# joaotavora/raytracing-one-weekend

Hardware: AMD Instinct MI355X
Metric: Msamples/sec (W×H×spp) on cover scene; achieved HBM GB/s vs peak (higher is better)
Workload: dtype f64

## Files before the change

### include/rtow.h

```cpp
#ifndef RTOW_H
#define RTOW_H

#include <stdint.h>

#ifdef __cplusplus
extern "C" {
#endif

#define RTOW_ABI_VERSION 9

#define RTOW_OK 0
#define RTOW_EINVAL (-1)
#define RTOW_ENODEV (-2)
#define RTOW_EHIP (-3)
#define RTOW_ENOSCENE (-4)
#define RTOW_EEMPTY (-5)
#define RTOW_ENOMEM (-6)

#define RTOW_MAT_LAMBERTIAN 0
#define RTOW_MAT_METAL 1
#define RTOW_MAT_DIELECTRIC 2

#define RTOW_PRIM_SPHERE 0
#define RTOW_PRIM_MOVING_SPHERE 1
// ... 51 lines not shown
  const int32_t *prim_index;
} rtow_scene_t;

typedef struct rtow_config_t {
  int32_t image_width;
  int32_t image_height;
  int32_t samples_per_pixel;
  int32_t nstreams;
  int32_t max_child_rays;
  int32_t precision;
  int32_t kernel;
  int32_t rank;
  int32_t nranks;
  int32_t tile_rows;
  uint64_t seed;
  int32_t stream_first;
  int32_t stream_count;
  int32_t accumulate;
  int32_t pad_;
} rtow_config_t;

typedef struct rtow_stats_t {
  uint64_t samples;
  uint64_t segments;
  uint64_t prim_tests;
  uint64_t node_tests;
  double kernel_ms;
  double total_ms;
  int32_t local_rows;
  int32_t kernel_used;
} rtow_stats_t;

typedef struct rtow_ctx rtow_ctx;

int rtow_abi_version(void);
const char *rtow_last_error(void);

int rtow_ctx_create(int device_id, rtow_ctx **out);
void rtow_ctx_destroy(rtow_ctx *ctx);

int rtow_scene_upload(rtow_ctx *ctx, const rtow_scene_t *scene);

#define RTOW_BUILDER_HOST_SAH 0
#define RTOW_BUILDER_DEVICE_LBVH 1
#define RTOW_BUILDER_AUTO 2
int rtow_ctx_set_builder(rtow_ctx *ctx, int32_t builder);

typedef struct rtow_build_info_t {
  int32_t builder;
  int32_t bvh_nodes;
  int32_t bvh_image_bytes;
  int32_t grid_image_bytes;
  double bvh_build_ms;
  double grid_build_ms;
  double upload_ms;
  int32_t bvh4_nodes;
  int32_t bvh4_image_bytes;
  int32_t ref_tree_nodes;
  int32_t bvh4_node_bytes;
  double ref_tree_stupid_volume;
  double ref_tree_build_ms;
} rtow_build_info_t;
int rtow_build_info(rtow_ctx *ctx, rtow_build_info_t *out);

int rtow_local_rows(const rtow_config_t *cfg);
int rtow_local_row_list(const rtow_config_t *cfg, int32_t *rows_out, int32_t capacity);

int rtow_render_device(rtow_ctx *ctx, const rtow_config_t *cfg, void *d_rgb_sums,
                       void *hip_stream, rtow_stats_t *stats);

int rtow_render_device_rgb8(rtow_ctx *ctx, const rtow_config_t *cfg, void *d_rgb8, void *hip_stream,
                            rtow_stats_t *stats);

int rtow_tonemap_device(rtow_ctx *ctx, const void *d_rgb_sums, int64_t n_values, int32_t spp_effective,
                        void *d_rgb8, void *hip_stream);

int rtow_profile_collect(rtow_ctx *ctx, double *kernel_ms_sum, int32_t *launches);

int rtow_debug_counters(rtow_ctx *ctx, unsigned long long *out48);

int rtow_debug_schedule(rtow_ctx *ctx, const rtow_config_t *cfg, uint32_t *out_pairs, int32_t capacity_pairs);

int rtow_debug_last_spec(rtow_ctx *ctx, uint32_t *out_spec);

int rtow_debug_tile_order(const rtow_scene_t *scene, const rtow_config_t *cfg, uint32_t *table_out, unsigned char *empty_out,
                          int32_t capacity, int32_t *n_empty, int32_t *tile_w_log2, int32_t *tile_h_log2);

int rtow_debug_image(rtow_ctx *ctx, int32_t which, void *out, int64_t capacity, int64_t *size_out);

typedef struct rtow_ray_t {
  double origin[3];
  double time;
  double direction[3];
  double tmax;
} rtow_ray_t;

typedef struct rtow_hit_t {
  double t;
  double point[3];
  double normal[3];
  int32_t prim;
  int32_t kind;
  int32_t material;
  int32_t front_face;
} rtow_hit_t;

int rtow_intersect_device(rtow_ctx *ctx, int32_t precision, int32_t kernel, const void *d_rays, int64_t n_rays,
                          void *d_hits, void *hip_stream, rtow_stats_t *stats);
int rtow_intersect(rtow_ctx *ctx, int32_t precision, int32_t kernel, const rtow_ray_t *rays, int64_t n_rays,
                   rtow_hit_t *hits, rtow_stats_t *stats);

int rtow_occluded_device(rtow_ctx *ctx, int32_t precision, int32_t kernel, const void *d_rays, int64_t n_rays,
                         void *d_occluded , void *hip_stream, rtow_stats_t *stats);
int rtow_occluded(rtow_ctx *ctx, int32_t precision, int32_t kernel, const rtow_ray_t *rays, int64_t n_rays,
                  uint8_t *occluded, rtow_stats_t *stats);

#define RTOW_MAX_HITS 8
int rtow_first_hits_device(rtow_ctx *ctx, int32_t precision, int32_t kernel, const void *d_rays, int64_t n_rays,
                           int32_t max_hits, void *d_hits ,
                           void *d_counts , void *hip_stream, rtow_stats_t *stats);
int rtow_first_hits(rtow_ctx *ctx, int32_t precision, int32_t kernel, const rtow_ray_t *rays, int64_t n_rays,
                    int32_t max_hits, rtow_hit_t *hits, int32_t *counts , rtow_stats_t *stats);

typedef struct rtow_point_query_t {
  double point[3];
  double time;
  double max_dist;
  double pad_;
} rtow_point_query_t;

typedef struct rtow_point_hit_t {
  double dist;
  double point[3];
  int32_t prim;
  int32_t kind;
  int32_t material;
  int32_t pad_;
} rtow_point_hit_t;

int rtow_closest_point_device(rtow_ctx *ctx, int32_t precision, int32_t kernel, const void *d_queries, int64_t n,
                              void *d_hits, void *hip_stream, rtow_stats_t *stats);
int rtow_closest_point(rtow_ctx *ctx, int32_t precision, int32_t kernel, const rtow_point_query_t *queries, int64_t n,
                       rtow_point_hit_t *hits, rtow_stats_t *stats);

#define RTOW_MAX_NEAREST 8
int rtow_nearest_device(rtow_ctx *ctx, int32_t precision, int32_t kernel, const void *d_queries, int64_t n,
                        int32_t k, void *d_hits , void *d_counts ,
                        void *hip_stream, rtow_stats_t *stats);
int rtow_nearest(rtow_ctx *ctx, int32_t precision, int32_t kernel, const rtow_point_query_t *queries, int64_t n,
                 int32_t k, rtow_point_hit_t *hits, int32_t *counts , rtow_stats_t *stats);

typedef struct rtow_radiance_params_t {
  uint64_t seed;
  int32_t samples_per_ray;
  int32_t max_child_rays;
  uint32_t sample_first;
  int32_t pad_;
} rtow_radiance_params_t;

int rtow_radiance_device(rtow_ctx *ctx, int32_t precision, int32_t kernel, const rtow_radiance_params_t *params,
                         const void *d_rays, int64_t n_rays, const void *d_ids ,
                         void *d_rgb_sums , void *hip_stream, rtow_stats_t *stats);
int rtow_radiance(rtow_ctx *ctx, int32_t precision, int32_t kernel, const rtow_radiance_params_t *params,
                  const rtow_ray_t *rays, int64_t n_rays, const uint32_t *ids, double *rgb_sums, rtow_stats_t *stats);

typedef struct rtow_guide_t {
// ... 83 lines not shown
```

### raytracing-one-weekend_amd/csrc/rtow_capi.cpp

```cpp

#include "rtow_ctx.h"

namespace {

thread_local std::string g_err;

template <class F>
int guarded(const char *what, F &&f) noexcept {
  try {
    return f();
  } catch (const std::bad_alloc &) {
    return fail(RTOW_ENOMEM, "%s: out of host memory", what);
  } catch (const std::exception &e) {
    return fail(RTOW_EINVAL, "%s: %s", what, e.what());
  } catch (...) {
    return fail(RTOW_EINVAL, "%s: unknown C++ exception", what);
  }
}

}
namespace rtow {
int set_last_error(int code, const char *fmt, ...) {
  char buf[512];
  va_list ap;
// ... 703 lines not shown
  P.local_rows = rows;
  P.seed_lo = (uint32_t)cfg->seed;
  P.seed_hi = (uint32_t)(cfg->seed >> 32);
  P.n_items = (uint32_t)n_items;
  P.n_lanes = (uint32_t)n_lanes;
  P.npix_local = (uint32_t)npix;
  P.div_npix = make_fastdiv((uint32_t)npix);
  P.div_w = make_fastdiv((uint32_t)cfg->image_width);
  P.div_tile = make_fastdiv((uint32_t)cfg->tile_rows);
  P.div_ns = make_fastdiv((uint32_t)streams_now);
  uint32_t th = 0, tw = 0;
  if (!c->knobs.no_tiles) tile_shape(cfg, rows, th, tw);
  P.tile_h_log2 = th;
  P.tile_w_log2 = tw;
  P.div_tpr_n = th ? (uint32_t)cfg->image_width >> tw : 1u;
  P.div_tpr = make_fastdiv(P.div_tpr_n);
  P.n_tile_rows = th ? (uint32_t)rows >> th : 1u;
  P.tile_table = nullptr;
  P.n_items_first = P.n_items;
  P.empty_batch = 64u;
  if (th) {
    const uint32_t sky_rows = P.n_tile_rows * (uint32_t)c->knobs.sky_eighths / 8u;
    const long long key[10] = {1, c->scene_gen, cfg->image_width, cfg->image_height, cfg->rank, cfg->nranks, cfg->tile_rows,
                               (long long)th, (long long)sky_rows, c->knobs.tile_order ? 1 : 0};
    if (std::memcmp(key, c->tile_key, sizeof key) != 0) {
      std::vector<unsigned char> empty;
      std::vector<uint32_t> table;
      if (c->knobs.tile_order) tile_classify(c->host_scene, cfg, th, tw, rows, empty);
      c->tile_empty = tile_queue_table(empty, c->knobs.tile_order, P.div_tpr_n, P.n_tile_rows, sky_rows, table);
      if ((rc = c->tile_table.ensure(table.size() * sizeof(uint32_t)))) return rc;
      c->tile_key[0] = -1;
      HIPCHK(hipStreamSynchronize(st));
      HIPCHK(hipMemcpy(c->tile_table.p, table.data(), table.size() * sizeof(uint32_t), hipMemcpyHostToDevice));
      std::memcpy(c->tile_key, key, sizeof key);
    }
    P.tile_table = (const uint32_t *)c->tile_table.p;
    P.n_items_first = P.n_items - c->tile_empty * 64u * (uint32_t)streams_now;
    P.empty_batch = 64u * (uint32_t)c->knobs.empty_levels;
  }
  P.partials = (double *)c->partials.p;
  P.stack = (uint32_t *)c->stack.p;
  P.spill = (uint32_t *)c->spill.p;
  P.spec = rtow::kSpecGeneric;
  if (kernel == RTOW_KERNEL_GRID && lds_bytes > 0 && !f32 && !c->knobs.no_spec && scene.n_tri == 0) {
    if (scene.n_mov == 0 && c->grid_fat_stride == 48u) P.spec = rtow::kSpecStaticSpheres;
    if (scene.n_mov > 0 && c->grid_fat_stride == 80u) P.spec = rtow::kSpecMovingSpheres;
    if (P.spec != rtow::kSpecGeneric && c->grid_ny == 1 && !c->knobs.no_flat) P.spec |= rtow::kSpecFlatY;
  }
  P.walk = c->grid_walk;
  P.b4_trips = c->knobs.bvh4_sm ? 0u : 1u;
  {
    const bool b4 = kernel == RTOW_KERNEL_BVH4;
    const bool b4_nodes_resident = b4 && scene.b4_lds_limit >= scene.b4_off_tri;
    int cap = c->knobs.walk_cap, open = c->knobs.walk_max_open;
    if (cap < 0) {
      cap = b4 ? 4 : 3;
      open = b4 ? (b4_nodes_resident ? 24 : 32) : 16;
    }
    if (cap > 0 && !b4) cap = std::max(cap, 3);
    P.walk_cap = cap > 0 ? (uint32_t)cap : 0xffffffffu;
    P.walk_max_open = (uint32_t)open;
    P.leaf_votes = (uint32_t)(c->knobs.leaf_votes > 0 ? c->knobs.leaf_votes : (b4 ? 28 : 16));
  }
  P.fetch_votes = (uint32_t)(c->knobs.fetch_votes > 0 ? c->knobs.fetch_votes : (kernel == RTOW_KERNEL_BVH4 ? 2 : 4));
  P.sm4_restart = (uint32_t)c->knobs.sm4_votes[0];
  P.sm4_scatter = (uint32_t)c->knobs.sm4_votes[1];
  P.sm4_leaf = (uint32_t)c->knobs.sm4_votes[2];
  P.counters = (unsigned long long *)c->counters.p;
  P.t_origin = P.counters + 16;

  if (st != nullptr) HIPCHK(hipStreamWaitEvent(st, c->upload_ev, 0));
  if (stats) HIPCHK(hipEventRecord(c->call_ev[0], st));
  if (!c->counters_init.p) {
    std::vector<unsigned long long> init(48, 0ull);
    init[5] = init[16] = ~0ull;
    if ((rc = c->counters_init.ensure(48 * sizeof(unsigned long long)))) return rc;
    HIPCHK(hipMemcpy(c->counters_init.p, init.data(), 48 * sizeof(unsigned long long), hipMemcpyHostToDevice));
  }
  HIPCHK(hipMemcpyAsync(c->counters.p, c->counters_init.p, 48 * sizeof(unsigned long long), hipMemcpyDeviceToDevice, st));
  const int slot = c->ev_count < kEventRing ? c->ev_count : -1;
  if (slot >= 0) HIPCHK(hipEventRecord(c->ev[slot][0], st));
  int launch_kernel = kernel;
  if (image_kernel && lds_bytes > 0 && c->knobs.stamps) launch_kernel = kernel + 16;
  int lrc = strict ? rtow::launch_trace_strict(P, launch_kernel, (int)grid, block, lds_bytes, st)
            : f32  ? rtow::launch_trace_f32(P, launch_kernel, (int)grid, block, lds_bytes, st)
                   : rtow::launch_trace_fast(P, launch_kernel, (int)grid, block, lds_bytes, st);
#ifdef RTOW_TAILSTAT
  if (const char *path = std::getenv("RTOW_TAILSTAT_OUT")) {
    HIPCHK(hipStreamSynchronize(st));
    std::vector<unsigned long long> ts((size_t)n_lanes / 64 * 8);
    HIPCHK(hipMemcpy(ts.data(), c->spill.p, ts.size() * 8, hipMemcpyDeviceToHost));
    if (FILE *f = std::fopen(path, "wb")) {
      std::fwrite(ts.data(), 8, ts.size(), f);
      std::fclose(f);
    }
  }
#endif
  if (lrc != 0) return fail(RTOW_EHIP, "trace kernel launch failed: %s", hipGetErrorString((hipError_t)lrc));
  c->last_spec = (int64_t)P.spec;
  if (slot >= 0) {
    HIPCHK(hipEventRecord(c->ev[slot][1], st));
    c->ev_count++;
  }
  rtow::ReduceParams R;
  R.partials = P.partials;
  R.out = (double *)d_rgb_sums;
  R.npix3 = (uint32_t)(npix * 3);
  R.nstreams = streams_now;
  R.accumulate = accumulate;
  R.W = (uint32_t)cfg->image_width;
  R.tile_w_log2 = tw;
  R.tile_h_log2 = th;
  R.tiles_per_row = P.div_tpr_n;
  R.rgb8 = nullptr;
  R.spp = 0.0;
  if (c->fuse_rgb8 && lvl_first == 0 && lvl_count == plan.count && !accumulate) {
    R.rgb8 = c->fuse_rgb8;
    R.spp = c->fuse_spp;
    c->fuse_used = true;
  }
  lrc = rtow::launch_reduce(R, st);
  if (lrc != 0) return fail(RTOW_EHIP, "reduce kernel launch failed: %s", hipGetErrorString((hipError_t)lrc));

  if (stats) {
    HIPCHK(hipEventRecord(c->call_ev[1], st));
    HIPCHK(hipMemcpyAsync(c->h_counters, c->counters.p, 48 * sizeof(unsigned long long),
                          hipMemcpyDeviceToHost, st));
    HIPCHK(hipStreamSynchronize(st));
    if (c->h_counters[47] != 0ull) {
      (void)check_dropped(c, false);
      return fail(RTOW_EHIP, "trace kernel: end-of-launch bound reached, %llu lanes gave up their samples",
                  c->h_counters[47]);
    }
    float ms = 0.f;
    HIPCHK(hipEventElapsedTime(&ms, c->call_ev[0], c->call_ev[1]));
    stats->total_ms = ms;
    if (slot >= 0) {
      HIPCHK(hipEventElapsedTime(&ms, c->ev[slot][0], c->ev[slot][1]));
      stats->kernel_ms = ms;
    }
    stats->samples = npix * ((unsigned long long)spt * (unsigned long long)(streams_now - 1) + (unsigned long long)spt_last);
    stats->segments = c->h_counters[1];
    if (kernel == RTOW_KERNEL_BRUTE) {
      stats->prim_tests = stats->segments * (unsigned long long)c->n_prims;
      stats->node_tests = 0;
    } else {
      stats->prim_tests = c->h_counters[2];
      stats->node_tests = c->h_counters[3];
    }
  }
  return RTOW_OK;
}

constexpr int64_t kMaxQueryRays = (1ll << 31) - 64;

static int query_map(rtow_ctx *c, int which, const int32_t **out) {
  if (c->q_map_ok[which]) {
    *out = (const int32_t *)c->q_map[which].p;
    return RTOW_OK;
  }
  const int ns = c->ds.n_sph, nm = c->ds.n_mov, nt = c->ds.n_tri, np = c->n_prims;
  const rtow_ctx::HostSceneCopy &h = c->host_scene;
  std::vector<int32_t> cls2ins((size_t)np);
  for (int i = 0; i < np; ++i) cls2ins[i] = i;
  if (h.have_order)
    for (int i = 0; i < np; ++i) {
      const int k = h.pk[i];
      const int base = k == RTOW_PRIM_SPHERE ? 0 : (k == RTOW_PRIM_MOVING_SPHERE ? ns : ns + nm);
      cls2ins[(size_t)base + h.pi[i]] = i;
    }
  std::vector<int32_t> table;
  if (which == 0) {
    table.swap(cls2ins);
  } else {
    std::vector<int32_t> matched;
    if (!c->rf.ready)
      if (int rc = match_slots(c, which, matched)) return rc;
    const std::vector<int32_t> &slot2tri = c->rf.ready ? c->rf.slot2tri[which - 1] : matched;
    table.assign((size_t)nt, -1);
    for (int k = 0; k < nt; ++k) table[(size_t)k] = cls2ins[(size_t)ns + nm + slot2tri[(size_t)k]];
  }
  DevBuf &b = c->q_map[which];
// ... 422 lines not shown
  HIPCHK(hipSetDevice(c->device));
  if ((rc = c->q_rays.ensure((size_t)n * sizeof(rtow_ray_t))) || (ids && (rc = c->q_ids.ensure((size_t)n * 8)))) return rc;
  if ((rc = camera_rays_device(c, cfg, c->q_rays.p, ids ? c->q_ids.p : nullptr, nullptr))) return rc;
  HIPCHK(hipMemcpy(rays, c->q_rays.p, (size_t)n * sizeof(rtow_ray_t), hipMemcpyDeviceToHost));
  if (ids) HIPCHK(hipMemcpy(ids, c->q_ids.p, (size_t)n * 8, hipMemcpyDeviceToHost));
  return RTOW_OK;
}

static int guides_device(rtow_ctx *c, const rtow_config_t *cfg, void *d_guides, void *hip_stream, rtow_stats_t *stats) {
  if (!c) return fail(RTOW_EINVAL, "ctx is NULL");
  CameraCall k;
  int rc;
  if ((rc = camera_call(cfg, k))) return rc;
  const long long tiles = (((long long)cfg->image_width + 7) / 8) * (((long long)k.rows + 7) / 8);
  if (tiles * 64 > 0xfffffff0LL) return fail(RTOW_EINVAL, "too many pixels (%lld)", k.npix);
  if (k.npix > 0 && !d_guides) return fail(RTOW_EINVAL, "NULL guide buffer");
  if (((uintptr_t)d_guides & 15u) != 0u) return fail(RTOW_EINVAL, "guide buffer must be 16-byte aligned");
  QueryRun q;
  if ((rc = query_begin(c, cfg->precision, cfg->kernel, stats, q))) return rc;
  if (stats) stats->local_rows = k.rows;
  if (k.npix == 0) return RTOW_OK;
  if (k.samples == 0) {
    HIPCHK(hipMemsetAsync(d_guides, 0, (size_t)k.npix * sizeof(rtow_guide_t), (hipStream_t)hip_stream));
    if (stats) HIPCHK(hipStreamSynchronize((hipStream_t)hip_stream));
    return RTOW_OK;
  }
  q.block_cap = c->knobs.guides_blocks;

  const int kernel = q.kernel;
  const int block = q.shape.block;
  const unsigned lds = q.shape.lds_bytes;
  const int build = q.strict ? 0 : 1;
  rtow::GuidesLaunchFn *const launch[2] = {rtow::launch_guides_strict, rtow::launch_guides_fast};
  rtow::QueryOccupancyFn *const occupancy[2] = {rtow::guides_occupancy_strict, rtow::guides_occupancy_fast};
  const int occ = occupancy[build](kernel, block, lds, nullptr);
  rc = query_launch(c, q, tiles * 64, occ, hip_stream, stats, [&](const rtow::TraceParams &P0, unsigned long long *counters, int grid) {
    rtow::TraceParams P = P0;
    camera_params(c, cfg, k, P);
    return launch[build](P, d_guides, (uint32_t)(tiles * 64), k.sample_first, (int32_t)k.samples, counters, kernel, grid, block,
                         lds, hip_stream);
  });
  if (rc == RTOW_OK && stats) {
    stats->samples = stats->segments = (uint64_t)k.npix * (uint64_t)k.samples;
    if (kernel == RTOW_KERNEL_BRUTE) stats->prim_tests = stats->segments * (uint64_t)c->n_prims;
  }
  return rc;
}

static int guides_host(rtow_ctx *c, const rtow_config_t *cfg, rtow_guide_t *guides, rtow_stats_t *stats) {
  if (!c) return fail(RTOW_EINVAL, "ctx is NULL");
  CameraCall k;
  int rc;
  if ((rc = camera_call(cfg, k))) return rc;
  if (k.npix > 0 && !guides) return fail(RTOW_EINVAL, "NULL guide array");
  if (k.npix == 0) return guides_device(c, cfg, nullptr, nullptr, stats);
  if (!c->have_scene) return fail(RTOW_ENOSCENE, "no scene uploaded");
  HIPCHK(hipSetDevice(c->device));
  if ((rc = c->q_guides.ensure((size_t)k.npix * sizeof(rtow_guide_t)))) return rc;
  if ((rc = guides_device(c, cfg, c->q_guides.p, nullptr, stats))) return rc;
  HIPCHK(hipMemcpy(guides, c->q_guides.p, (size_t)k.npix * sizeof(rtow_guide_t), hipMemcpyDeviceToHost));
  return RTOW_OK;
}
static_assert(sizeof(rtow_guide_t) == 64, "rtow_guide_t is four 16-byte stores");

int64_t rtow_camera_ray_count(const rtow_config_t *cfg) {
  CameraCall k;
  if (int rc = camera_call(cfg, k)) return rc;
  return (int64_t)(k.npix * k.samples);
}

int rtow_debug_counters(rtow_ctx *c, unsigned long long *out48) {
  if (!c || !out48) return fail(RTOW_EINVAL, "NULL argument");
  if (!c->counters.p) return fail(RTOW_ENOSCENE, "no launch yet");
  HIPCHK(hipSetDevice(c->device));
  HIPCHK(hipDeviceSynchronize());
  HIPCHK(hipMemcpy(out48, c->counters.p, 48 * sizeof(unsigned long long), hipMemcpyDeviceToHost));
  return RTOW_OK;
}

int rtow_debug_last_spec(rtow_ctx *c, uint32_t *out_spec) {
  if (!c || !out_spec) return fail(RTOW_EINVAL, "NULL argument");
  if (c->last_spec < 0) return fail(RTOW_ENOSCENE, "no launch yet");
  *out_spec = (uint32_t)c->last_spec;
  return RTOW_OK;
}

int rtow_tonemap_device(rtow_ctx *c, const void *d_rgb_sums, int64_t n_values, int32_t spp_effective,
                        void *d_rgb8, void *hip_stream) {
  if (!c) return fail(RTOW_EINVAL, "ctx is NULL");
  if (!d_rgb_sums || !d_rgb8) return fail(RTOW_EINVAL, "NULL device pointer");
  if (n_values < 0 || n_values > 0xffffffffLL) return fail(RTOW_EINVAL, "n_values out of range");
  if (spp_effective <= 0) return fail(RTOW_EINVAL, "spp_effective must be positive");
  HIPCHK(hipSetDevice(c->device));
  int lrc = rtow::launch_tonemap((const double *)d_rgb_sums, (unsigned char *)d_rgb8, (uint32_t)n_values,
                                 (double)spp_effective, hip_stream);
  if (lrc != 0) return fail(RTOW_EHIP, "tonemap launch failed: %s", hipGetErrorString((hipError_t)lrc));
  return RTOW_OK;
}

int rtow_profile_collect(rtow_ctx *c, double *kernel_ms_sum, int32_t *launches) {
  if (!c) return fail(RTOW_EINVAL, "ctx is NULL");
  HIPCHK(hipSetDevice(c->device));
  double sum = 0.0;
  for (int i = 0; i < c->ev_count; ++i) {
    HIPCHK(hipEventSynchronize(c->ev[i][1]));
    float ms = 0.f;
    HIPCHK(hipEventElapsedTime(&ms, c->ev[i][0], c->ev[i][1]));
    sum += ms;
  }
  if (kernel_ms_sum) *kernel_ms_sum = sum;
  if (launches) *launches = c->ev_count;
  const bool waited = c->ev_count > 0;
  c->ev_count = 0;
  return waited ? check_dropped(c, false) : RTOW_OK;
}

static int impl_render(rtow_ctx *c, const rtow_scene_t *scene, const rtow_config_t *cfg, double *rgb_sums_host,
                rtow_stats_t *stats) {
  if (!c) return fail(RTOW_EINVAL, "ctx is NULL");
  if (!rgb_sums_host) return fail(RTOW_EINVAL, "rgb_sums_host is NULL");
  int rc = validate_cfg(cfg);
  if (rc) return rc;
  if ((rc = upload_for(c, scene, cfg))) return rc;
  const int rows = rtow_local_rows(cfg);
  const size_t bytes = (size_t)rows * cfg->image_width * 3 * sizeof(double);
  if (bytes == 0) {
    if (stats) {
      std::memset(stats, 0, sizeof *stats);
    }
    return RTOW_OK;
  }
  if ((rc = c->out.ensure(bytes))) return rc;
  void *d_out = c->out.p;
  if (cfg->accumulate)
    HIPCHK(hipMemcpy(d_out, rgb_sums_host, bytes, hipMemcpyHostToDevice));
  rc = rtow_render_device(c, cfg, d_out, nullptr, stats);
  if (rc != RTOW_OK) return rc;
  if ((rc = mirror_dropped(c, nullptr))) return rc;
  HIPCHK(hipMemcpy(rgb_sums_host, d_out, bytes, hipMemcpyDeviceToHost));
  return check_dropped(c, true);
}

static int impl_render_device_rgb8(rtow_ctx *c, const rtow_config_t *cfg, void *d_rgb8, void *hip_stream,
                                   rtow_stats_t *stats) {
  if (!c) return fail(RTOW_EINVAL, "ctx is NULL");
  if (!d_rgb8) return fail(RTOW_EINVAL, "d_rgb8 is NULL");
  int rc = validate_cfg(cfg);
  if (rc) return rc;
  const int spp_eff = cfg->samples_per_pixel / cfg->nstreams * cfg->nstreams;
  if (spp_eff <= 0) return fail(RTOW_EINVAL, "no effective samples (samples_per_pixel < nstreams)");
  if (cfg->accumulate) return fail(RTOW_EINVAL, "the rgb8 entry points own their sums: accumulate must be 0");
  const int rows = rtow_local_rows(cfg);
  const size_t n = (size_t)rows * cfg->image_width * 3;
  if (n == 0) {
    if (stats) std::memset(stats, 0, sizeof *stats);
    return RTOW_OK;
  }
  HIPCHK(hipSetDevice(c->device));
  if ((rc = c->out.ensure(n * sizeof(double)))) return rc;
  c->fuse_rgb8 = (unsigned char *)d_rgb8;
  c->fuse_spp = (double)spp_eff;
  c->fuse_used = false;
  rc = impl_render_device(c, cfg, c->out.p, hip_stream, stats);
  c->fuse_rgb8 = nullptr;
  if (rc == RTOW_OK && !c->fuse_used) rc = rtow_tonemap_device(c, c->out.p, (int64_t)n, spp_eff, d_rgb8, hip_stream);
  return rc;
// ... 168 lines not shown
```

### raytracing-one-weekend_amd/csrc/rtow_ctx.h

```cpp
#pragma once
#include <hip/hip_runtime.h>

#include <cmath>
#include <cstdarg>
#include <cstdio>
#include <cstdlib>
#include <algorithm>
#include <chrono>
#include <cstring>
#include <string>
#include <vector>

#include "../../include/rtow.h"
#include "rtow_bvh.h"
#include "rtow_bvh4.h"
#include "rtow_device.h"
#include "rtow_grid.h"
#include "rtow_reftree.h"

namespace rtow {
int set_last_error(int code, const char *fmt, ...);
template <class... A>
inline int fail(int code, const char *fmt, A... a) {
  return set_last_error(code, fmt, a...);
// ... 8 lines not shown
      return fail(RTOW_EHIP, "%s: %s (%s:%d)", #expr, hipGetErrorString(e_), __FILE__, __LINE__); \
  } while (0)

constexpr unsigned kLdsLimit = 160u * 1024u;
constexpr int kEventRing = 256;

namespace rtow {

struct DevBuf {
  void *p = nullptr;
  size_t bytes = 0;
  int ensure(size_t need) {
    if (need <= bytes) return RTOW_OK;
    if (p) {
      HIPCHK(hipFree(p));
      p = nullptr;
      bytes = 0;
    }
    size_t want = need + need / 8 + 256;
    HIPCHK(hipMalloc(&p, want));
    bytes = want;
    return RTOW_OK;
  }
  void release() {
    if (p) (void)hipFree(p);
    p = nullptr;
    bytes = 0;
  }
};

struct PinnedArena {
  unsigned char *p = nullptr;
  size_t cap = 0, used = 0;
};
int h2d_block(void *dst, const void *src, size_t n);

template <class T>
int upload(DevBuf &b, const std::vector<T> &v) {
  const size_t n = v.size() * sizeof(T);
  if (int rc = b.ensure(n ? n : sizeof(T))) return rc;
  return n ? h2d_block(b.p, v.data(), n) : RTOW_OK;
}

inline double now_ms() {
  using namespace std::chrono;
  return duration<double, std::milli>(steady_clock::now().time_since_epoch()).count();
}

}
using rtow::DevBuf;
using rtow::PinnedArena;
using rtow::h2d_block;
using rtow::now_ms;
using rtow::upload;

struct Knobs {
  int bvh_leaf = 0;
  double bvh_ct = -1.0;
  bool no_leaf_order = false;
  double grid_cpp = 1.0;
  double grid_large = 4.0;
  int grid_max_tris = 8192;
  unsigned long long partials_cap = 8ull << 30;
  int bvh_block = 0;
  int blocks_per_cu = 0;
  bool no_tiles = false;
  int sky_eighths = 1;
  bool stamps = false;
  bool bvh4_no_aux = false;
  bool no_bvh4 = false;
  int fetch_votes = 0;
  int leaf_votes = 0;
  int walk_cap = -1, walk_max_open = 0;
  bool bvh4_sm = false;
  int sm4_votes[3] = {8, 16, 16};
  int bvh4_stack_k = 0;
  int sched_chunk = 10;
  int sched_chunk_mesh = 16;
  int ploc_radius = -1;
  int device_tree = 2;
  bool stream_scalar = false;
  bool no_spec = false;
  bool no_flat = false;
  bool tile_order = true;
  int empty_levels = 3;
  int tail_bound = 0;
  int radiance_blocks = 0;
  int guides_blocks = 0;
  void read() {
    auto geti = [](const char *n, int d) { const char *e = std::getenv(n); return e ? std::atoi(e) : d; };
    auto getd = [](const char *n, double d) { const char *e = std::getenv(n); return e ? std::atof(e) : d; };
    bvh_leaf = geti("RTOW_BVH_LEAF", 0);
    bvh_ct = getd("RTOW_BVH_CT", -1.0);
    no_leaf_order = std::getenv("RTOW_NO_LEAF_ORDER") != nullptr;
    grid_cpp = getd("RTOW_GRID_CPP", 1.0);
    grid_large = getd("RTOW_GRID_LARGE", 4.0);
    grid_max_tris = geti("RTOW_GRID_MAX_TRIS", 8192);
    if (const char *e = std::getenv("RTOW_PARTIALS_MAX_MB")) partials_cap = (unsigned long long)std::atoll(e) << 20;
    bvh_block = geti("RTOW_BVH_BLOCK", 0);
    if (bvh_block != 256 && bvh_block != 512 && bvh_block != 1024) bvh_block = 0;
    blocks_per_cu = geti("RTOW_BLOCKS_PER_CU", 0);
    if (blocks_per_cu < 1 || blocks_per_cu > 16) blocks_per_cu = 0;
    no_tiles = std::getenv("RTOW_NO_TILES") != nullptr;
    sky_eighths = std::min(std::max(geti("RTOW_SKY_EIGHTHS", 1), 0), 8);
    stamps = std::getenv("RTOW_STAMPS") != nullptr;
    no_bvh4 = std::getenv("RTOW_NO_BVH4") != nullptr;
    bvh4_no_aux = std::getenv("RTOW_BVH4_NO_AUX") != nullptr;
    fetch_votes = std::min(std::max(geti("RTOW_FETCH_VOTES", 0), 0), 64);
    leaf_votes = std::min(std::max(geti("RTOW_LEAF_VOTES", 0), 0), 64);
    bvh4_sm = std::getenv("RTOW_BVH4_SM") != nullptr;
    if (const char *e = std::getenv("RTOW_WALK_CAP")) {
      int a = 0, b = 0;
      if (std::sscanf(e, "%d,%d", &a, &b) == 2 && a > 0 && b > 0) {
        walk_cap = a;
        walk_max_open = std::min(b, 64);
      } else {
        walk_cap = 0;
      }
    }
    if (const char *e = std::getenv("RTOW_SM4_VOTES")) {
      int a = 0, b = 0, d = 0;
      if (std::sscanf(e, "%d,%d,%d", &a, &b, &d) == 3) {
        sm4_votes[0] = std::min(std::max(a, 1), 64);
        sm4_votes[1] = std::min(std::max(b, 1), 64);
        sm4_votes[2] = std::min(std::max(d, 1), 64);
      }
    }
    bvh4_stack_k = std::min(std::max(geti("RTOW_BVH4_STACK_K", 0), 0), 64);
    sched_chunk = std::min(std::max(geti("RTOW_SCHED_CHUNK", 10), 0), 4096);
    sched_chunk_mesh = std::min(std::max(geti("RTOW_SCHED_CHUNK_MESH", 16), 0), 4096);
    tail_bound = std::max(geti("RTOW_TAIL_BOUND", 0), 0);
    radiance_blocks = std::max(geti("RTOW_RADIANCE_BLOCKS", 0), 0);
    guides_blocks = std::max(geti("RTOW_GUIDES_BLOCKS", 0), 0);
    tile_order = geti("RTOW_TILE_ORDER", 1) != 0;
    empty_levels = std::min(std::max(geti("RTOW_EMPTY_LEVELS", 3), 1), 16);
    no_spec = std::getenv("RTOW_NO_SPEC") != nullptr;
    no_flat = std::getenv("RTOW_NO_FLAT") != nullptr;
    stream_scalar = std::getenv("RTOW_STREAM_SCALAR") != nullptr;
    if (const char *e = std::getenv("RTOW_PLOC_RADIUS")) ploc_radius = std::min(std::max(std::atoi(e), 0), 64);
    if (const char *e = std::getenv("RTOW_DEVICE_TREE"))
      device_tree = std::strcmp(e, "radix") == 0 ? 0 : (std::strcmp(e, "ploc") == 0 ? 1 : 2);
    if (ploc_radius >= 0 && !std::getenv("RTOW_DEVICE_TREE")) device_tree = ploc_radius == 0 ? 0 : 1;
  }
};

constexpr unsigned kNeedBvh = 1u, kNeedGrid = 2u, kNeedF32 = 4u, kNeedBvh4 = 8u, kNeedAll = 15u;

struct rtow_ctx {
  int device = 0;
  Knobs knobs;
  int num_cus = 0;
  bool have_scene = false;
  rtow::DevScene ds{};
  rtow::DevCamera cam{};
  int n_prims = 0;
  DevBuf sph, sph_r, mov, tri, tri16, prim_mat, mats, blob, cam_dev, gblob;
  DevBuf blob4;
  bool have_bvh4 = false;
  bool have_tri16 = false;
  int bvh4_depth = 0;
  DevBuf blob32, gblob32, cam32_dev;
  rtow::DevScene ds32{};
  uint32_t gblob_bytes = 0;
  uint32_t grid_fat_stride = 0;
  int32_t grid_ny = 0;
  GridWalkConsts grid_walk{};
  int64_t last_spec = -1;
  bool have_grid = false;
  uint32_t blob_bytes = 0;
  long long bvh_nodes = 0;
  int builder = RTOW_BUILDER_HOST_SAH;
  int builder_req = RTOW_BUILDER_AUTO;
  void *lbvh_scratch = nullptr;
  void *grid_scratch = nullptr;
  rtow_build_info_t build_info{};
  struct HostSceneCopy {
    std::vector<double> sg, mg, tg;
    std::vector<int32_t> pk, pi;
    bool have_order = false;
    rtow_camera_t cam{};
  } host_scene;
  DevBuf tile_table;
  long long tile_key[10] = {-1, 0, 0, 0, 0, 0, 0, 0, 0, 0};
  uint32_t tile_empty = 0;
  long long scene_gen = 0;
  DevBuf rtree;
  bool have_rtree = false;
  PinnedArena arena;
  unsigned built = 0;
  DevBuf partials, stack, counters, spill;
  DevBuf out, out8;
  unsigned char *fuse_rgb8 = nullptr;
  double fuse_spp = 0.0;
  bool fuse_used = false;
  DevBuf counters_init;
  DevBuf dropped;
  unsigned long long *h_dropped = nullptr;
  hipEvent_t upload_ev = nullptr;
  int occ[3][5] = {{0, 0, 0, 0, 0}, {0, 0, 0, 0, 0}, {0, 0, 0, 0, 0}};
  hipEvent_t ev[kEventRing][2] = {};
  int ev_count = 0;
  hipEvent_t call_ev[2] = {};
  unsigned long long *h_counters = nullptr;
  DevBuf q_counters, q_spill, q_rays, q_hits, q_occ, q_map[3];
  DevBuf q_stack, q_ids, q_rgb;
  DevBuf q_guides;
  DevBuf q_khits, q_kcounts;
  bool q_map_ok[3] = {false, false, false};
  hipEvent_t q_ev[4] = {};
  unsigned long long *h_qcounters = nullptr;
  struct Refit {
    bool ready = false;
    std::vector<int32_t> slot2tri[2];
    DevBuf map2, map4, par2, par4, need4, flags, nbox2, nbox4, sbox4, pbox, partials;
    DevBuf area;
    DevBuf g_sph, g_mov, g_tri;
    int refits = 0;
    double refit_ms = 0.0;
    hipEvent_t ev[2] = {};
  } rf;
};

static uint32_t bvh4_min_stack(const rtow_ctx *c) { return c->knobs.bvh4_stack_k > 0 ? (uint32_t)c->knobs.bvh4_stack_k : 6u; }

namespace rtow {
void lbvh_release(void *handle);
void grid_build_release(void *handle);
int validate_scene(const rtow_scene_t *s);
int impl_scene_upload(rtow_ctx *c, const rtow_scene_t *s);
int upload_for(rtow_ctx *c, const rtow_scene_t *scene, const rtow_config_t *cfg);
int impl_scene_refit(rtow_ctx *c, const rtow_scene_t *s);
int match_slots(rtow_ctx *c, int which, std::vector<int32_t> &slot2tri);
}
using rtow::impl_scene_refit;
using rtow::impl_scene_upload;
using rtow::match_slots;
using rtow::upload_for;
using rtow::validate_scene;
```

### raytracing-one-weekend_amd/csrc/rtow_device.h

```cpp
#pragma once
#include <stdint.h>

#include "rtow_walk_consts.h"

namespace rtow {

struct DevMaterial {
  double att[3];
  double fuzz;
  double ir;
  int32_t kind;
  int32_t pad_;
};

struct DevCamera {
  double origin[3], u[3], v[3];
  double horizontal[3], vertical[3], llc[3];
  double lens_radius, t0, t1;
};

struct DevScene {
  const double *sph;
  const double *sph_r;
  const double *mov;
// ... 21 lines not shown
  uint32_t b4_aux_src, b4_aux_lds;
  uint32_t b4_stack_base;
  uint32_t b4_stack_k;
  double b4_c[3];
  float b4_is[3];
  uint32_t b4_half;
  const unsigned char *rtree;
  uint32_t rt_off_ids;
};
constexpr uint32_t kRefNodeBytes = 64;
constexpr uint32_t kRefLeafFlag = 0x80000000u;
constexpr int kRefStackDepth = 48;

struct FastDiv {
  uint32_t magic, shift;
};

struct alignas(64) FetchDecode {
  uint32_t tile_w_log2, tile_h_log2;
  const uint32_t *tile_table;
  FastDiv div_ns;
  FastDiv div_tpr;
  uint32_t div_tpr_n;
  int32_t nstreams;
  FastDiv div_tile;
  int32_t rank, nranks, tile_rows;
  uint32_t sample_base;
  int32_t spt;
  int32_t spt_last;
  uint32_t npix_local;
};
struct alignas(32) FetchHead {
  uint32_t n_items;
  uint32_t n_items_first;
  uint32_t empty_batch;
  int32_t W;
  double *partials;
  unsigned long long *counters;
};
static_assert(sizeof(FetchDecode) == 128 && sizeof(FetchHead) == 32, "aligned runs: one or two wide scalar loads each");

struct TraceParams : FetchDecode, FetchHead {
  DevScene sc;
  const DevCamera *cam;
  const float *cam32;
  int32_t H;
  int32_t stream_first;
  uint32_t tail_bound;
  double inv_wm1, inv_hm1;
  int32_t max_child_rays;
  int32_t local_rows;
  uint32_t seed_lo, seed_hi;
  uint32_t n_lanes;
  FastDiv div_npix, div_w;
  uint32_t n_tile_rows;
  uint32_t *stack;
  uint32_t *spill;
  uint32_t spec;
  uint32_t b4_trips;
  uint32_t fetch_votes;
  uint32_t leaf_votes;
  uint32_t walk_cap, walk_max_open;
  uint32_t sm4_restart, sm4_scatter, sm4_leaf;
  unsigned long long *dropped;
  unsigned long long *t_origin;
  GridWalkConsts walk;
};

constexpr uint32_t kSpecGeneric = 0u, kSpecStaticSpheres = 1u, kSpecMovingSpheres = 2u;
constexpr uint32_t kSpecFlatY = 4u;

struct ReduceParams {
  const double *partials;
  double *out;
  uint32_t npix3;
  int32_t nstreams;
  int32_t accumulate;
  uint32_t W, tile_w_log2, tile_h_log2, tiles_per_row;
  unsigned char *rgb8;
  double spp;
};

int launch_trace_strict(const TraceParams &p, int kernel, int grid, int block, unsigned lds_bytes,
                        void *stream);
int launch_trace_fast(const TraceParams &p, int kernel, int grid, int block, unsigned lds_bytes,
                      void *stream);
int launch_trace_f32(const TraceParams &p, int kernel, int grid, int block, unsigned lds_bytes,
                     void *stream);
int trace_occupancy_strict(int kernel, int block, unsigned lds_bytes);
int trace_occupancy_fast(int kernel, int block, unsigned lds_bytes);
int trace_occupancy_f32(int kernel, int block, unsigned lds_bytes);
int launch_reduce(const ReduceParams &p, void *stream);
int launch_tonemap(const double *sums, unsigned char *rgb8, uint32_t n, double spp, void *stream);
int launch_place_rows(const void *gathered, void *image, uint32_t n_ranks, uint32_t max_rows, uint32_t row_bytes,
                      uint32_t height, uint32_t tile_rows, void *stream);

}
```

### raytracing-one-weekend_amd/csrc/rtow_scene.cpp

```cpp

#include "rtow_ctx.h"
#include "rtow_scene_records.h"

namespace rtow {
int lbvh_build(const double *sph, const double *sph_r, const double *mov, const double *tri, int ns, int nm,
               int nt, double time0, double time1, const double cam_origin[3], int leaf_max, void *stream,
               void **handle, int *n_nodes, int ploc_radius);
int lbvh_emit(void *handle, int leaf_max, unsigned char *blob_dev, uint32_t off_ids, int n_nodes, void *stream);
int lbvh_bvh4_collapse(void *handle, int leaf_max, void *stream, int *n_nodes, int *depth, float root_box[6]);
int lbvh_bvh4_emit(void *handle, unsigned char *blob_dev, int half, const double map_c[3], const double map_s[3],
                   uint32_t off_tri, uint32_t off_pmat, const double *tri, const int32_t *prim_mat, void *stream);
struct GridBuildBounds {
  double gmn[3], gmx[3];
  double scale_prims;
  int32_t n_small, n_large;
};
int grid_build_phase1(const double *sph, const double *sph_r, const double *mov, const double *tri, int ns, int nm,
                      int nt, double time0, double time1, double large_ratio, void *stream, void **handle,
                      GridBuildBounds *out);
int grid_build_phase2(void *handle, const float gminf[3], const float cellf[3], const int32_t n[3], double pad,
                      void *stream, unsigned long long *total_ids, unsigned long long *max_list);
int grid_build_phase3(void *handle, const float gminf[3], const float cellf[3], const int32_t n[3], double pad,
                      unsigned long long total_ids, unsigned char *blob_dev, uint32_t off_cells, uint32_t off_ids,
                      void *stream, const double *sph, uint32_t off_fat, const double *mov, int ns, uint32_t fat_stride);
// ... 91 lines not shown
    dc.v[i] = k.v[i];
    dc.horizontal[i] = k.horizontal[i];
    dc.vertical[i] = k.vertical[i];
    dc.llc[i] = k.lower_left_corner[i];
  }
  dc.lens_radius = k.lens_radius;
  dc.t0 = k.t0;
  dc.t1 = k.t1;
}

static void scene_materials(const rtow_scene_t *s, rtow::SceneRecords &rec) {
  const int ns = s->n_spheres, nm = s->n_moving, nt = s->n_triangles;
  std::vector<int32_t> &pmat = rec.pmat;
  pmat.resize((size_t)ns + nm + nt);
  for (int i = 0; i < ns; ++i) pmat[i] = s->sphere_mat[i];
  for (int i = 0; i < nm; ++i) pmat[(size_t)ns + i] = s->moving_mat[i];
  for (int i = 0; i < nt; ++i) pmat[(size_t)ns + nm + i] = s->triangle_mat[i];
  rec.mats_bytes.resize((size_t)s->n_materials * sizeof(rtow::DevMaterial));
  for (int i = 0; i < s->n_materials; ++i) {
    const rtow_material_t &m = s->materials[i];
    rtow::DevMaterial d;
    std::memset(&d, 0, sizeof d);
    const bool diel = m.kind == RTOW_MAT_DIELECTRIC;
    for (int k = 0; k < 3; ++k) d.att[k] = diel ? 1.0 : m.albedo[k];
    d.fuzz = m.kind == RTOW_MAT_LAMBERTIAN ? 0.0 : m.fuzz;
    d.ir = m.ir;
    d.kind = m.kind;
    std::memcpy(&rec.mats_bytes[(size_t)i * sizeof d], &d, sizeof d);
  }
}

static rtow::SceneRecords make_scene_records(const rtow_scene_t *s) {
  rtow::SceneRecords rec;
  rtow::geometry_records(s->sphere_geom, s->n_spheres, s->moving_geom, s->n_moving, s->triangle_geom, s->n_triangles, rec);
  scene_materials(s, rec);
  return rec;
}


constexpr uint32_t kSkip = ~0u;
struct RecordOffsets {
  uint32_t sph, mov, tri, pmat, mats;
};
static int copy_record_sections(unsigned char *dst, const RecordOffsets &o, const rtow_ctx *c, int ns, int nm, int nt, int np,
                                size_t mats_n) {
  const struct {
    uint32_t off;
    const void *src;
    size_t n;
  } parts[] = {{o.sph, c->sph.p, (size_t)ns * 32}, {o.mov, c->mov.p, (size_t)nm * 64}, {o.tri, c->tri.p, (size_t)nt * 96},
               {o.pmat, c->prim_mat.p, (size_t)np * 4}, {o.mats, c->mats.p, mats_n}};
  for (const auto &p : parts)
    if (p.off != kSkip && p.n) HIPCHK(hipMemcpyAsync(dst + p.off, p.src, p.n, hipMemcpyDeviceToDevice, nullptr));
  return RTOW_OK;
}
static hipError_t d2d(void *dst, const void *src, size_t n) {
  return n ? hipMemcpyAsync(dst, src, n, hipMemcpyDeviceToDevice, nullptr) : hipSuccess;
}

static void bvh4_set_frame(rtow_ctx *c, const double map_c[3], const double map_s[3]) {
  for (rtow::DevScene *d : {&c->ds, &c->ds32})
    for (int k = 0; k < 3; ++k) {
      d->b4_c[k] = map_c[k];
      d->b4_is[k] = (float)(1.0 / map_s[k]);
    }
}

static void bvh4_resident(rtow_ctx *c, const rtow::Bvh4Image &img4, size_t bytes) {
  c->have_bvh4 = img4.ok;
  c->build_info.bvh4_nodes = img4.ok ? img4.n_nodes : 0;
  c->build_info.bvh4_image_bytes = img4.ok ? (int32_t)bytes : 0;
  c->build_info.bvh4_node_bytes = img4.ok ? (int32_t)img4.node_bytes() : 0;
  if (!img4.ok) return;
  c->bvh4_depth = img4.depth;
  c->ds.blob4 = (const unsigned char *)c->blob4.p;
  c->ds.blob4_bytes = (uint32_t)bytes;
  c->ds.b4_off_tri = img4.off_tri;
  c->ds.b4_off_pmat = img4.off_pmat;
  c->ds.b4_off_mats = img4.off_mats;
  c->ds.b4_half = img4.half ? 1u : 0u;
  bvh4_set_frame(c, img4.map_c, img4.map_s);
}

static void grid_resident(rtow_ctx *c, const rtow::GridImage &gimg) {
  c->have_grid = gimg.ok;
  c->grid_fat_stride = (gimg.ok && gimg.off_fat) ? gimg.fat_stride : 0u;
  c->grid_ny = gimg.ok ? gimg.n[1] : 0;
  c->grid_walk = gimg.ok ? make_grid_walk_consts(gimg.header, gimg.off_ids, gimg.off_cells) : GridWalkConsts{};
  c->gblob_bytes = gimg.ok ? (uint32_t)gimg.total_bytes : 0u;
  rtow::DevScene &ds = c->ds;
  ds.gblob = (const unsigned char *)c->gblob.p;
  ds.gblob_bytes = c->gblob_bytes;
  ds.g_off_sph = gimg.off_sph;
  ds.g_off_mov = gimg.off_mov;
  ds.g_off_tri = gimg.off_tri;
  ds.g_off_pmat = gimg.off_pmat;
  ds.g_off_mats = gimg.off_mats;
  for (rtow::DevScene *d : {&c->ds, &c->ds32}) {
    d->g_off_cells = gimg.off_cells;
    d->g_off_ids = gimg.off_ids;
  }
}

static void image32_resident(rtow::DevScene &d32, bool grid, const Image32 *im, const void *dev, size_t bytes) {
  (grid ? d32.gblob : d32.blob) = im ? (const unsigned char *)dev : nullptr;
  (grid ? d32.gblob_bytes : d32.blob_bytes) = im ? (uint32_t)bytes : 0u;
  if (!im) return;
  (grid ? d32.g_off_sph : d32.off_sph) = im->off_sph;
  (grid ? d32.g_off_mov : d32.off_mov) = im->off_mov;
  (grid ? d32.g_off_tri : d32.off_tri) = im->off_tri;
  (grid ? d32.g_off_sph32 : d32.off_sph32) = im->off_sph32;
  (grid ? d32.g_off_mov32 : d32.off_mov32) = im->off_mov32;
  (grid ? d32.g_off_pmat : d32.off_pmat) = im->off_pmat;
  (grid ? d32.g_off_mats : d32.off_mats) = im->off_mats;
}

static int camera_resident(rtow_ctx *c, const rtow_camera_t &cam, bool f32) {
  camera_record(cam, c->cam);
  int rc;
  if ((rc = c->cam_dev.ensure(sizeof c->cam)) || (rc = h2d_block(c->cam_dev.p, &c->cam, sizeof c->cam))) return rc;
  if (!f32) return RTOW_OK;
  const double *cd = reinterpret_cast<const double *>(&c->cam);
  float cam32[21];
  for (int i = 0; i < 21; ++i) cam32[i] = (float)cd[i];
  if ((rc = c->cam32_dev.ensure(sizeof cam32))) return rc;
  return h2d_block(c->cam32_dev.p, cam32, sizeof cam32);
}

static int host_scene_copy(rtow_ctx *c, const rtow_scene_t *s, bool with_order) {
  rtow_ctx::HostSceneCopy &h = c->host_scene;
  h.sg.assign(s->sphere_geom, s->sphere_geom + 4 * (size_t)s->n_spheres);
  h.mg.assign(s->moving_geom, s->moving_geom + 8 * (size_t)s->n_moving);
  h.tg.assign(s->triangle_geom, s->triangle_geom + 9 * (size_t)s->n_triangles);
  h.cam = s->camera;
  if (!with_order) return RTOW_OK;
  h.have_order = s->prim_kind && s->prim_index;
  if (h.have_order) {
    for (int i = 0; i < s->n_prims; ++i) {
      const int k = s->prim_kind[i], ix = s->prim_index[i];
      const int cnt = k == RTOW_PRIM_SPHERE ? s->n_spheres : k == RTOW_PRIM_MOVING_SPHERE ? s->n_moving
                      : k == RTOW_PRIM_TRIANGLE ? s->n_triangles : -1;
      if (ix < 0 || ix >= cnt) return fail(RTOW_EINVAL, "prim_kind / prim_index entry %d out of range", i);
    }
    h.pk.assign(s->prim_kind, s->prim_kind + s->n_prims);
    h.pi.assign(s->prim_index, s->prim_index + s->n_prims);
  } else {
    h.pk.clear();
    h.pi.clear();
  }
  return RTOW_OK;
}

enum class Invalidate { Upload, Refit };
static void invalidate_resident(rtow_ctx *c, Invalidate what) {
  c->scene_gen++;
  c->have_rtree = false;
  for (auto &o : c->occ) o[0] = o[1] = o[2] = o[3] = o[4] = 0;
  c->q_map_ok[1] = c->q_map_ok[2] = false;
  if (what == Invalidate::Refit) return;
  c->q_map_ok[0] = false;
  c->rf.ready = false;
  c->rf.refits = 0;
  c->rf.refit_ms = 0.0;
  c->build_info.ref_tree_nodes = 0;
  c->build_info.ref_tree_stupid_volume = 0.0;
}

static int grid_device_build(rtow_ctx *c, const rtow_camera_t &cam, const rtow::SceneRecords &rec, rtow::GridImage &gimg) {
  const std::vector<double> &sph = rec.sph, &mov = rec.mov, &tri = rec.tri;
  const int ns = (int)(sph.size() / 4), nm = (int)(mov.size() / 8), nt = (int)(tri.size() / 12);
  const double cpp = c->knobs.grid_cpp;
  const double large_ratio = c->knobs.grid_large;
  int rc;
  rtow::GridBuildBounds gb;
  int grc = rtow::grid_build_phase1((const double *)c->sph.p, (const double *)c->sph_r.p, (const double *)c->mov.p,
                                    (const double *)c->tri.p, ns, nm, nt, cam.t0, cam.t1, large_ratio,
                                    nullptr, &c->grid_scratch, &gb);
  if (grc) return fail(RTOW_EHIP, "device grid build failed (phase 1, stage %d): %s", grc, hipGetErrorString(hipGetLastError()));
  if (gb.n_small <= 0 || gb.n_large > 64) return RTOW_OK;
  rtow::GridHeader hd;
  rtow::grid_header(gb.gmn, gb.gmx, gb.scale_prims, cam.origin, (size_t)gb.n_small, cpp, hd);
  unsigned long long total_ids = 0, max_list = 0;
  grc = rtow::grid_build_phase2(c->grid_scratch, hd.gminf, hd.cellf, hd.n, hd.pad, nullptr, &total_ids, &max_list);
  if (grc) return fail(RTOW_EHIP, "device grid build failed (phase 2, stage %d): %s", grc, hipGetErrorString(hipGetLastError()));
// ... 188 lines not shown
static void publish_dev_scene(rtow_ctx *c, const rtow_scene_t *s, const TreeImages &t) {
  const rtow::SceneImage &img = t.img;
  c->blob_bytes = (uint32_t)img.total_bytes;
  c->bvh_nodes = img.n_nodes;
  rtow::DevScene &ds = c->ds;
  ds.sph = (const double *)c->sph.p;
  ds.sph_r = (const double *)c->sph_r.p;
  ds.mov = (const double *)c->mov.p;
  ds.tri = (const double *)c->tri.p;
  ds.tri16 = c->have_tri16 ? (const double *)c->tri16.p : nullptr;
  ds.prim_mat = (const int32_t *)c->prim_mat.p;
  ds.mats = (const rtow::DevMaterial *)c->mats.p;
  ds.n_sph = s->n_spheres;
  ds.n_mov = s->n_moving;
  ds.n_tri = s->n_triangles;
  ds.n_mats = s->n_materials;
  ds.blob = (const unsigned char *)c->blob.p;
  ds.blob_bytes = c->blob_bytes;
  ds.off_ids = img.off_ids;
  ds.off_sph = img.off_sph;
  ds.off_mov = img.off_mov;
  ds.off_tri = img.off_tri;
  ds.off_pmat = img.off_pmat;
  ds.off_mats = img.off_mats;
  ds.n_nodes = img.n_nodes;
  ds.leaf_direct = t.leaf_direct ? 1 : 0;
  c->n_prims = s->n_spheres + s->n_moving + s->n_triangles;
}

static int build_f32_images(rtow_ctx *c, const rtow::SceneRecords &rec, const TreeImages &t, const rtow::GridImage &gimg,
                            bool grid_on_device) {
  int rc;
  const bool device_tree = c->builder == RTOW_BUILDER_DEVICE_LBVH;
  Image32 b32;
  make_image32(device_tree ? nullptr : t.img.blob.data(), t.img.off_sph, rec.sph, rec.mov, t.leaf_direct ? t.tri_img : rec.tri,
               t.leaf_direct ? t.pmat_img : rec.pmat, rec.mats_bytes, b32);
  if ((rc = upload(c->blob32, b32.blob))) return rc;
  if (device_tree)
    HIPCHK(hipMemcpy(c->blob32.p, c->blob.p, t.img.off_sph, hipMemcpyDeviceToDevice));
  image32_resident(c->ds32, false, &b32, c->blob32.p, b32.blob.size());
  if (!gimg.ok) {
    image32_resident(c->ds32, true, nullptr, nullptr, 0);
    return RTOW_OK;
  }
  Image32 g32;
  make_image32(grid_on_device ? nullptr : gimg.blob.data(), gimg.off_sph, rec.sph, rec.mov, rec.tri, rec.pmat, rec.mats_bytes, g32);
  if ((rc = upload(c->gblob32, g32.blob))) return rc;
  if (grid_on_device)
    HIPCHK(hipMemcpy(c->gblob32.p, c->gblob.p, gimg.off_sph, hipMemcpyDeviceToDevice));
  image32_resident(c->ds32, true, &g32, c->gblob32.p, g32.blob.size());
  return RTOW_OK;
}

static int scene_upload(rtow_ctx *c, const rtow_scene_t *s, unsigned need) {
  if (!c) return fail(RTOW_EINVAL, "ctx is NULL");
  int rc = validate_scene(s);
  if (rc) return rc;
  HIPCHK(hipSetDevice(c->device));
  HIPCHK(hipDeviceSynchronize());
  if (!c->arena.p) {
    if (hipHostMalloc((void **)&c->arena.p, 8u << 20, hipHostMallocDefault) == hipSuccess)
      c->arena.cap = 8u << 20;
    else
      c->arena.p = nullptr;
  }
  ArenaScope arena_scope(&c->arena);
  if (need & kNeedF32) need |= kNeedBvh | kNeedGrid;
  c->built = 0;
  c->have_scene = false;
  invalidate_resident(c, Invalidate::Upload);
  const double t_up0 = now_ms();
  if ((rc = host_scene_copy(c, s, true))) return rc;
  const rtow::SceneRecords rec = make_scene_records(s);
  if ((rc = upload_record_arrays(c, rec, need))) return rc;
  const double t_bvh0 = now_ms();
  TreeImages trees;
  if ((rc = build_tree_images(c, s, rec, need, trees))) return rc;
  const double t_bvh1 = now_ms();
  rtow::GridImage gimg;
  bool grid_on_device = false;
  if ((rc = build_grid(c, s->camera, rec, need, gimg, grid_on_device))) return rc;
  const double t_grid1 = now_ms();
  if (gimg.ok && !grid_on_device && (rc = upload(c->gblob, gimg.blob))) return rc;
  grid_resident(c, gimg);
  publish_dev_scene(c, s, trees);
  c->ds32 = c->ds;
  if ((need & kNeedF32) && (rc = build_f32_images(c, rec, trees, gimg, grid_on_device))) return rc;
  if ((rc = camera_resident(c, s->camera, (need & kNeedF32) != 0))) return rc;
  HIPCHK(hipEventRecord(c->upload_ev, nullptr));
  c->built = need;
  c->have_scene = true;
  rtow_build_info_t &bi = c->build_info;
  bi.builder = c->builder;
  bi.bvh_nodes = (int32_t)trees.img.n_nodes;
  bi.bvh_image_bytes = (int32_t)c->blob_bytes;
  bi.grid_image_bytes = (int32_t)c->gblob_bytes;
  bi.bvh_build_ms = t_bvh1 - t_bvh0;
  bi.grid_build_ms = t_grid1 - t_bvh1;
  bi.upload_ms = now_ms() - t_up0;
  return RTOW_OK;
}

namespace rtow {

int validate_scene(const rtow_scene_t *s) {
  if (!s) return fail(RTOW_EINVAL, "scene is NULL");
  if (s->n_spheres < 0 || s->n_moving < 0 || s->n_triangles < 0 || s->n_materials < 0)
    return fail(RTOW_EINVAL, "negative count in scene");
  const long long np = (long long)s->n_spheres + s->n_moving + s->n_triangles;
  if (np == 0) return fail(RTOW_EEMPTY, "scene has no primitives");
  if (s->n_prims != np) return fail(RTOW_EINVAL, "n_prims (%d) != sum of classes (%lld)", s->n_prims, np);
  if (s->n_materials == 0 || !s->materials) return fail(RTOW_EINVAL, "scene has no materials");
  if ((s->n_spheres && (!s->sphere_geom || !s->sphere_mat)) ||
      (s->n_moving && (!s->moving_geom || !s->moving_mat)) ||
      (s->n_triangles && (!s->triangle_geom || !s->triangle_mat)))
    return fail(RTOW_EINVAL, "NULL geometry/material array");
  auto chk = [&](const int32_t *m, int n) {
    for (int i = 0; i < n; ++i)
      if (m[i] < 0 || m[i] >= s->n_materials) return false;
    return true;
  };
  if (!chk(s->sphere_mat, s->n_spheres) || !chk(s->moving_mat, s->n_moving) ||
      !chk(s->triangle_mat, s->n_triangles))
    return fail(RTOW_EINVAL, "material index out of range");
  for (int i = 0; i < s->n_materials; ++i)
    if (s->materials[i].kind < 0 || s->materials[i].kind > 2)
      return fail(RTOW_EINVAL, "material %d has unknown kind %d", i, s->materials[i].kind);
  return RTOW_OK;
}

int impl_scene_upload(rtow_ctx *c, const rtow_scene_t *s) {
  if (c && c->builder_req == RTOW_BUILDER_AUTO) c->builder = RTOW_BUILDER_HOST_SAH;
  return scene_upload(c, s, kNeedAll);
}

int upload_for(rtow_ctx *c, const rtow_scene_t *scene, const rtow_config_t *cfg) {
  if (!c) return fail(RTOW_EINVAL, "ctx is NULL");
  int rc = validate_scene(scene);
  if (rc) return rc;
  const long long np = (long long)scene->n_spheres + scene->n_moving + scene->n_triangles;
  unsigned need;
  const int k = cfg->kernel;
  const bool mesh = scene->n_spheres == 0 && scene->n_moving == 0 && scene->n_triangles > 0 && !c->knobs.no_bvh4;
  if (cfg->precision == RTOW_F32)
    need = kNeedAll;
  else if (k == RTOW_KERNEL_REFTREE || k == RTOW_KERNEL_BRUTE || (k == RTOW_KERNEL_AUTO && np <= 16))
    need = 0u;
  else if ((k == RTOW_KERNEL_AUTO || k == RTOW_KERNEL_GRID) && scene->n_triangles == 0)
    need = kNeedGrid;
  else if (k == RTOW_KERNEL_GRID)
    need = kNeedGrid | kNeedBvh;
  else if (mesh && (k == RTOW_KERNEL_AUTO || k == RTOW_KERNEL_BVH4))
    need = kNeedBvh4;
  else
    need = kNeedBvh;
  if (c->builder_req == RTOW_BUILDER_AUTO) {
    const bool device = mesh && need == kNeedBvh4 && scene->n_triangles >= 16384;
    c->builder = device ? RTOW_BUILDER_DEVICE_LBVH : RTOW_BUILDER_HOST_SAH;
  }
  rc = scene_upload(c, scene, need);
  if (rc == RTOW_OK && (need & kNeedGrid) && !(need & kNeedBvh) && !c->have_grid)
    rc = scene_upload(c, scene, need | kNeedBvh);
  if (rc == RTOW_OK && need == kNeedBvh4 && !c->have_bvh4)
    rc = scene_upload(c, scene, kNeedBvh);
  return rc;
}

// ... 158 lines not shown
      (rc = r.g_tri.ensure((size_t)nt * 72 + 8)))
    return rc;
  if ((ns && (rc = h2d_block(r.g_sph.p, s->sphere_geom, (size_t)ns * 32))) ||
      (nm && (rc = h2d_block(r.g_mov.p, s->moving_geom, (size_t)nm * 64))) ||
      (nt && (rc = h2d_block(r.g_tri.p, s->triangle_geom, (size_t)nt * 72))) ||
      (rc = h2d_block(c->prim_mat.p, rec.pmat.data(), (size_t)np * 4)) ||
      (rc = h2d_block(c->mats.p, rec.mats_bytes.data(), rec.mats_bytes.size())))
    return rc;
  auto *sph = (double *)c->sph.p, *sph_r = (double *)c->sph_r.p, *mov = (double *)c->mov.p, *tri = (double *)c->tri.p;
  if (rtow::refit_records((const double *)r.g_sph.p, (const double *)r.g_mov.p, (const double *)r.g_tri.p, ns, nm, nt, sph,
                          sph_r, mov, tri, c->have_tri16 ? (double *)c->tri16.p : nullptr, nullptr))
    return fail(RTOW_EHIP, "refit record pass failed: %s", hipGetErrorString(hipGetLastError()));
  if (((c->built & kNeedBvh) || c->have_bvh4) &&
      rtow::refit_prim_boxes(sph, sph_r, mov, tri, ns, nm, nt, s->camera.t0, s->camera.t1, (double *)r.pbox.p, nullptr))
    return fail(RTOW_EHIP, "refit box pass failed: %s", hipGetErrorString(hipGetLastError()));
  return RTOW_OK;
}

static int refit_bvh2_images(rtow_ctx *c, const rtow_camera_t &cam, size_t mats_n) {
  rtow_ctx::Refit &r = c->rf;
  const rtow::DevScene &ds = c->ds;
  const int ns = ds.n_sph, nm = ds.n_mov, nt = ds.n_tri, np = c->n_prims;
  const auto *sph = (const double *)c->sph.p, *mov = (const double *)c->mov.p, *tri = (const double *)c->tri.p;
  const auto *pmat_tri = (const int32_t *)c->prim_mat.p + ns + nm;
  const int32_t *map2 = ds.leaf_direct ? (const int32_t *)r.map2.p : nullptr;
  int rc;
  unsigned char *b = (unsigned char *)c->blob.p;
  if (map2 && rtow::refit_tri_section(nt, tri, pmat_tri, map2, b, ds.off_tri, ds.off_pmat, 0, nullptr))
    return fail(RTOW_EHIP, "refit record scatter failed: %s", hipGetErrorString(hipGetLastError()));
  const RecordOffsets all{ds.off_sph, ds.off_mov, ds.off_tri, ds.off_pmat, ds.off_mats};
  if ((rc = copy_record_sections(b, map2 ? RecordOffsets{kSkip, kSkip, kSkip, kSkip, ds.off_mats} : all, c, ns, nm, nt, np, mats_n)))
    return rc;
  if (rtow::refit_bvh2(b, ds.n_nodes, ds.off_ids, np, map2, ns + nm, (const double *)r.pbox.p, (const int32_t *)r.par2.p,
                       (uint32_t *)r.flags.p, (double *)r.nbox2.p, (double *)r.partials.p, 1, cam.origin,
                       (double *)r.area.p + 1, nullptr))
    return fail(RTOW_EHIP, "refit BVH pass failed: %s", hipGetErrorString(hipGetLastError()));
  if (!(c->built & kNeedF32)) return RTOW_OK;
  const rtow::DevScene &d32 = c->ds32;
  unsigned char *b32 = (unsigned char *)c->blob32.p;
  HIPCHK(d2d(b32, b, ds.off_sph));
  if ((rc = copy_record_sections(b32, {d32.off_sph, d32.off_mov, kSkip, map2 ? kSkip : d32.off_pmat, d32.off_mats}, c, ns, nm, nt,
                                 np, mats_n)))
    return rc;
  if (rtow::refit_tri_section(nt, tri, pmat_tri, map2, b32, d32.off_tri, map2 ? d32.off_pmat : ~0u, 1, nullptr) ||
      rtow::refit_spheres32(ns, nm, sph, mov, b32, d32.off_sph32, d32.off_mov32, nullptr))
    return fail(RTOW_EHIP, "refit f32 record scatter failed: %s", hipGetErrorString(hipGetLastError()));
  return RTOW_OK;
}

static int refit_bvh4_image(rtow_ctx *c, const rtow_camera_t &cam, size_t mats_n) {
  rtow_ctx::Refit &r = c->rf;
  const rtow::DevScene &ds = c->ds;
  const int ns = ds.n_sph, nm = ds.n_mov, nt = ds.n_tri;
  unsigned char *b4 = (unsigned char *)c->blob4.p;
  const int n4 = c->build_info.bvh4_nodes;
  const uint32_t nb = ds.b4_half ? rtow::kBvh4HalfNodeBytes : rtow::kBvh4NodeBytes, co = ds.b4_half ? 48u : 96u;
  double *frame_dev = (double *)r.area.p + 2;
  if (rtow::refit_tri_section(nt, (const double *)c->tri.p, (const int32_t *)c->prim_mat.p + ns + nm, (const int32_t *)r.map4.p,
                              b4, ds.b4_off_tri, ds.b4_off_pmat, 0, nullptr) ||
      rtow::refit_bvh4(b4, n4, nb, co, (int)ds.b4_half, nt, (const int32_t *)r.map4.p, ns + nm, (const double *)r.pbox.p,
                       (const int32_t *)r.par4.p, (const int32_t *)r.need4.p, (uint32_t *)r.flags.p, (double *)r.nbox4.p,
                       (double *)r.sbox4.p, cam.origin, frame_dev, nullptr))
    return fail(RTOW_EHIP, "refit 4-wide pass failed: %s", hipGetErrorString(hipGetLastError()));
  HIPCHK(d2d(b4 + ds.b4_off_mats, c->mats.p, mats_n));
  if (ds.b4_half) {
    double frame[6];
    HIPCHK(hipMemcpy(frame, frame_dev, sizeof frame, hipMemcpyDeviceToHost));
    bvh4_set_frame(c, frame, frame + 3);
  }
  return RTOW_OK;
}

static int refit_grid_images(rtow_ctx *c, const rtow_scene_t *s, rtow::SceneRecords &rec) {
  const int ns = c->ds.n_sph, nm = c->ds.n_mov, nt = c->ds.n_tri, np = c->n_prims;
  const size_t mats_n = rec.mats_bytes.size();
  int rc;
  rtow::GridImage gimg;
  if (nt <= c->knobs.grid_max_tris) {
    rtow::sphere_records(s->sphere_geom, ns, rec.sph, rec.sph_r);
    rec.mov.resize((size_t)nm * 8);
    rec.tri.resize((size_t)nt * 12);
    if ((rc = grid_device_build(c, s->camera, rec, gimg))) return rc;
  }
  grid_resident(c, gimg);
  if (!(c->built & kNeedF32)) return RTOW_OK;
  if (!gimg.ok) {
    image32_resident(c->ds32, true, nullptr, nullptr, 0);
    return RTOW_OK;
  }
  Image32 g32;
  const size_t total = layout_image32(gimg.off_sph, ns, nm, nt, np, mats_n, g32);
  if ((rc = c->gblob32.ensure(total))) return rc;
  unsigned char *g = (unsigned char *)c->gblob32.p;
  HIPCHK(hipMemsetAsync(g, 0, total, nullptr));
  HIPCHK(d2d(g, c->gblob.p, gimg.off_sph));
  if ((rc = copy_record_sections(g, {g32.off_sph, g32.off_mov, kSkip, g32.off_pmat, g32.off_mats}, c, ns, nm, nt, np, mats_n)))
    return rc;
  if (rtow::refit_tri_section(nt, (const double *)c->tri.p, nullptr, nullptr, g, g32.off_tri, ~0u, 1, nullptr) ||
      rtow::refit_spheres32(ns, nm, (const double *)c->sph.p, (const double *)c->mov.p, g, g32.off_sph32, g32.off_mov32, nullptr))
    return fail(RTOW_EHIP, "refit f32 grid records failed: %s", hipGetErrorString(hipGetLastError()));
  image32_resident(c->ds32, true, &g32, g, total);
  return RTOW_OK;
}

namespace rtow {
int impl_scene_refit(rtow_ctx *c, const rtow_scene_t *s) {
  if (!c) return fail(RTOW_EINVAL, "ctx is NULL");
  int rc = validate_scene(s);
  if (rc) return rc;
  if (!c->have_scene) return fail(RTOW_ENOSCENE, "no scene uploaded");
  if ((rc = refit_check_shape(c, s))) return rc;
  const double t_call = now_ms();
  HIPCHK(hipSetDevice(c->device));
  HIPCHK(hipDeviceSynchronize());
  rtow_ctx::Refit &r = c->rf;
  if (!r.ev[0])
    for (hipEvent_t &e : r.ev) HIPCHK(hipEventCreate(&e));
  HIPCHK(hipEventRecord(r.ev[0], nullptr));
  c->have_scene = false;
  ArenaScope arena_scope(&c->arena);
  if (!r.ready && (rc = refit_prepare(c))) return rc;
  SceneRecords rec;
  scene_materials(s, rec);
  if ((rc = refit_records_stage(c, s, rec))) return rc;
  if ((c->built & kNeedBvh) && (rc = refit_bvh2_images(c, s->camera, rec.mats_bytes.size()))) return rc;
  if (c->have_bvh4 && (rc = refit_bvh4_image(c, s->camera, rec.mats_bytes.size()))) return rc;
  if ((c->built & kNeedGrid) && (rc = refit_grid_images(c, s, rec))) return rc;
  if ((rc = camera_resident(c, s->camera, (c->built & kNeedF32) != 0))) return rc;
  if ((rc = host_scene_copy(c, s, false))) return rc;
  invalidate_resident(c, Invalidate::Refit);
  HIPCHK(hipEventRecord(r.ev[1], nullptr));
  HIPCHK(hipEventRecord(c->upload_ev, nullptr));
  c->have_scene = true;
  r.refits++;
  r.refit_ms = now_ms() - t_call;
  return RTOW_OK;
}
}

int rtow_refit_info(rtow_ctx *c, rtow_refit_info_t *out) {
  if (!c || !out) return fail(RTOW_EINVAL, "NULL argument");
  if (!c->have_scene) return fail(RTOW_ENOSCENE, "no scene uploaded");
  std::memset(out, 0, sizeof *out);
  HIPCHK(hipSetDevice(c->device));
  HIPCHK(hipDeviceSynchronize());
  const rtow_ctx::Refit &r = c->rf;
  out->refits = r.refits;
  out->grid_resident = c->have_grid ? 1 : 0;
  out->refit_ms = r.refit_ms;
  out->bvh_area_ratio = (c->built & kNeedBvh) ? 1.0 : 0.0;
  if (r.refits > 0) {
    float ms = 0.f;
    HIPCHK(hipEventElapsedTime(&ms, r.ev[0], r.ev[1]));
    out->device_ms = ms;
    if (c->built & kNeedBvh) {
      double a[2];
      HIPCHK(hipMemcpy(a, r.area.p, sizeof a, hipMemcpyDeviceToHost));
      out->bvh_area_ratio = a[0] > 0.0 ? a[1] / a[0] : 1.0;
    }
  }
  return RTOW_OK;
}
```

### raytracing-one-weekend_amd/csrc/rtow_trace_body.h

```cpp

#include <hip/hip_runtime.h>
#include <stdint.h>
#include <type_traits>

#include "rtow_device.h"

#ifndef RTOW_SUFFIX
#error "define RTOW_SUFFIX"
#endif
#define RTOW_CAT2(a, b) a##b
#define RTOW_CAT(a, b) RTOW_CAT2(a, b)

namespace rtow {
namespace {
#include "rtow_trace_math.h"
#include "rtow_trace_rng.h"
#include "rtow_trace_hit.h"
#include "rtow_trace_stamps.h"
#include "rtow_trace_bvh.h"
#include "rtow_trace_grid.h"
#include "rtow_trace_bvh4.h"
#ifndef RTOW_FAST_MATH
#include "rtow_trace_reftree.h"
#endif
// ... 114 lines not shown
    const uint32_t tc = tile - tr * kd.div_tpr_n;
    const uint32_t lr0 = tr << kd.tile_h_log2;
    const uint32_t q = fastdiv(lr0, FastDiv{kd.div_tile.magic, kd.div_tile.shift});
    const uint32_t gi0 = (q * (uint32_t)kd.nranks + (uint32_t)kd.rank) * (uint32_t)kd.tile_rows + (lr0 - q * (uint32_t)kd.tile_rows);
    const uint32_t item0 = k * npix_local + (tile << 6);
    const uint32_t j0 = tc << kd.tile_w_log2;
    const uint32_t s0 = kd.sample_base + k * (uint32_t)kd.spt;
    const int32_t cnt = k + 1u == (uint32_t)kd.nstreams ? kd.spt_last : kd.spt;
    if (g64 == ug) {
      ip.item = item0 + w;
      ip.j = j0 + (w & ((1u << kd.tile_w_log2) - 1u));
      ip.gi = gi0 + (w >> kd.tile_w_log2);
      ip.sample0 = s0;
      ip.count = cnt;
      break;
    }
  }
  return ip;
}

__device__ __forceinline__ void camera_ray(const TraceParams &P, Rng &g, uint32_t k0, uint32_t k1, uint32_t j,
                                           uint32_t gi, V3 &ro, V3 &rd, real &rtime) {
  g.r = 0u;
  const int from_top_i = P.H - (int)gi - 1;
  uint32_t o0, o1, o2, o3;
  philox4x32(g.r, g.sample, g.pixel, 0u, k0, k1, o0, o1, o2, o3);
  g.r += 1u;
  real ju, jv, jt, px, py;
  jitter_from_block(o0, o1, o2, ju, jv, jt);
  lens_from_block(o0, o1, o2, o3, px, py);
  const real u = fast_div((real)(int)j + ju, (real)(P.W - 1));
  const real v = fast_div((real)from_top_i + jv, (real)(P.H - 1));
#ifdef RTOW_REAL_F32
  const RTOW_CONST float *cm = (const RTOW_CONST float *)P.cam32;
#else
  cdptr cm = (cdptr)(const double *)P.cam;
#endif
  const real lens = cm[18], ct0 = cm[19], ct1 = cm[20];
  const real rdx = lens * px, rdy = lens * py;
  const V3 offset = V3{cm[3], cm[4], cm[5]} * rdx + V3{cm[6], cm[7], cm[8]} * rdy;
  const V3 from = V3{cm[0], cm[1], cm[2]} + offset;
  rd = V3{cm[15], cm[16], cm[17]} + u * V3{cm[9], cm[10], cm[11]} + v * V3{cm[12], cm[13], cm[14]} - from;
  ro = from;
  rtime = jt * (ct1 - ct0) + ct0;
}

__device__ __forceinline__ bool scatter_dir(Rng &g, uint32_t k0, uint32_t k1, int kind, real m_fuzz, real m_ir, V3 rd,
                                            V3 normal, bool front, V3 &dir) {
  uint32_t o0, o1, o2, o3;
  philox4x32(g.r, g.sample, g.pixel, 0u, k0, k1, o0, o1, o2, o3);
  g.r += 1u;
  V3 dirbase = {0, 0, 0};
  if (kind == 2) {
    const real ir = m_ir;
    const V3 unit = normalize(rd);
    const real cos_theta = dot(-unit, normal);
    const real sin_theta = fast_sqrt(real(1.0) - cos_theta * cos_theta);
    const real ratio = front ? fast_rcp(ir) : ir;
    bool refl = ratio * sin_theta > real(1.0);
    if (!refl) {
      real r0 = fast_div(real(1.0) - ratio, real(1.0) + ratio);
      r0 = r0 * r0;
      const real x = real(1.0) - cos_theta;
      const real x2 = x * x;
      const real R = r0 + (real(1.0) - r0) * (x2 * x2 * x);
      refl = R > coin_from_block(o0, o1, o3);
    }
    dirbase = refl ? reflect(unit, normal) : refract(unit, normal, ratio);
  } else if (kind == 1) {
    dirbase = reflect(rd, normal);
  }
  const V3 rnd = ball_from_block(o0, o1, o2, o3);
  bool absorbed = false;
  if (kind == 0) {
    absorbed = rabs(normal.x - rnd.x) < real(1e-8) && rabs(normal.y - rnd.y) < real(1e-8) &&
               rabs(normal.z - rnd.z) < real(1e-8);
    dir = normal + rnd;
  } else {
    dir = dirbase + m_fuzz * rnd;
  }
  return !absorbed;
}

template <int KERNEL, bool LDS, bool STAMPS = false, int SPEC = 0>
__global__ void __launch_bounds__(KERNEL >= 2 && KERNEL <= 4 ? 1024 : 256)
    RTOW_CAT(rtow_trace_, RTOW_SUFFIX)(const TraceParams P) {
  const DevScene &sc = P.sc;
  const uint32_t k0 = P.seed_lo, k1 = P.seed_hi;
  const unsigned lane = lane_id();
  [[maybe_unused]] const uint32_t lane_g = blockIdx.x * blockDim.x + threadIdx.x;

  Image<LDS> im;
  [[maybe_unused]] Bvh4Reader<LDS> im4;
  stage_scene<KERNEL, LDS>(sc, im, im4);

  bool done = false;
  bool need_sample = true;
  bool pending_hit = false;
  int s_left = 0;
  uint32_t item = 0xffffffffu;
  uint32_t j = 0;
  uint32_t gi = 0;
  V3d acc = {0.0, 0.0, 0.0};
  V3 ro = {0, 0, 0}, rd = {0, 0, 1};
  real rtime = 0;
  int depth = 0;
  [[maybe_unused]] int nb = 0;
#ifdef RTOW_FAST_MATH
  V3 throughput = {1, 1, 1};
#endif
  Rng g = {0, 0, 0};
  uint32_t nseg = 0, nnode = 0, nprim = 0;
  [[maybe_unused]] float t_resume = 0.0f;
  [[maybe_unused]] uint32_t w_cur = 0x1fffffu, w_sa = 0u;
  Closest best;
  best.t = 0;
  best.prim = -1;
  bool helping = false;
  bool holding = false;
  uint32_t partners = 0u;
  int n_out = 0;
  uint32_t tail_left = P.tail_bound;
  asm volatile("" : "+v"(tail_left));
  ItemPool pool;
  const uint32_t n_waves = (gridDim.x * blockDim.x) >> 6;
#ifdef RTOW_TAILSTAT
  unsigned long long ts_start = __builtin_amdgcn_s_memrealtime(), ts_empty = 0ull;
  uint32_t ts_trips = 0u, ts_trips_after = 0u, ts_live = 0u, ts_left = 0u, ts_pool = 0u;
#endif
  Stamps<STAMPS> stamps;
  stamps.start();
  unsigned long long t_empty = 0ull;
  unsigned long long trips_after_empty = 0ull;
  if constexpr (STAMPS) {
    if (lane == 0) atomicMin(P.t_origin, (unsigned long long)__builtin_amdgcn_s_memrealtime());
  }

  for (;;) {
    bool need_item = false;
    if (!done && need_sample && s_left <= 0) {
      if (helping) {
        helping = false;
        holding = true;
        done = true;
      } else if (n_out == 0) {
        need_item = true;
      }
    }
    unsigned long long need_mask = __ballot(need_item);
    if (need_mask != 0ull && (uint32_t)__popcll(need_mask) < P.fetch_votes && __ballot(!done && !need_item) != 0ull) {
      need_mask = 0ull;
      need_item = false;
    }
    if (need_mask != 0ull) {
      const RTOW_CONST TraceParams *kp = (const RTOW_CONST TraceParams *)__builtin_amdgcn_kernarg_segment_ptr();
      asm volatile("" : "+s"(kp));
      const FetchHead fh = load_fetch_head(kp);
      if (need_item && item != 0xffffffffu) {
        double *dst = fh.partials + (size_t)item * 3;
        dst[0] = acc.x;
        dst[1] = acc.y;
        dst[2] = acc.z;
        item = 0xffffffffu;
      }
      const unsigned long long mine = take_items(pool, need_mask, lane, n_waves, fh);
      if (need_item) {
        if (mine >= (unsigned long long)fh.n_items) {
          done = true;
#ifdef RTOW_TAILSTAT
          if (ts_empty == 0ull) ts_empty = 1ull;
#endif
          if constexpr (STAMPS) {
            if (t_empty == 0ull) t_empty = __builtin_amdgcn_s_memrealtime();
          }
        } else {
          const ItemPos ip = decode_item(kp, fh, (uint32_t)mine);
          item = ip.item;
          j = ip.j;
          gi = ip.gi;
          g.pixel = gi * (uint32_t)fh.W + j;
          g.sample = ip.sample0;
          s_left = ip.count;
          acc = {0.0, 0.0, 0.0};
        }
      }
    }
#ifdef RTOW_TAILSTAT
    {
      const bool first = __ballot(ts_empty == 1ull) != 0ull && __ballot(ts_empty > 1ull) == 0ull;
      if (first) {
        const unsigned long long now = __builtin_amdgcn_s_memrealtime();
        ts_live = (uint32_t)__popcll(__ballot(!done));
        uint32_t sl = (!done && s_left > 0) ? (uint32_t)s_left : 0u;
        for (int off = 32; off >= 1; off >>= 1) sl += __shfl_xor(sl, off);
        ts_left = sl;
// ... 282 lines not shown
      const real u = fast_div((real)(int)j + ju, (real)(P.W - 1));
      const real v = fast_div((real)from_top_i + jv, (real)(P.H - 1));
#endif
#ifdef RTOW_REAL_F32
      const RTOW_CONST float *cm = (const RTOW_CONST float *)P.cam32;
#else
      cdptr cm = (cdptr)(const double *)P.cam;
#endif
      const real lens = cm[18], ct0 = cm[19], ct1 = cm[20];
      real px, py;
      {
        const uint32_t q = s_b >> 30;
        const real cx = (q & 1u) ? s_sn : s_cs, sy = (q & 1u) ? s_cs : s_sn;
        px = s_sq * ((q == 1u || q == 2u) ? -cx : cx);
        py = s_sq * (q >= 2u ? -sy : sy);
      }
      const real rdx = lens * px, rdy = lens * py;
      const V3 offset = V3{cm[3], cm[4], cm[5]} * rdx + V3{cm[6], cm[7], cm[8]} * rdy;
      const V3 from = V3{cm[0], cm[1], cm[2]} + offset;
      rd = V3{cm[15], cm[16], cm[17]} + u * V3{cm[9], cm[10], cm[11]} + v * V3{cm[12], cm[13], cm[14]} - from;
      ro = from;
      rtime = jt * (ct1 - ct0) + ct0;
      depth = P.max_child_rays;
      nb = 0;
#ifdef RTOW_FAST_MATH
      throughput = {1, 1, 1};
#endif
      need_sample = false;
    }
    if (do_scat) {
      pending_hit = false;
      bool absorbed = false;
      const real s_r = (real)max(max(o2 & 0xffffu, o2 >> 16), o3 & 0xffffu) * real(0x1p-16);
      const real s_rs = s_r * s_sq;
      const V3 rnd = V3{s_rs * s_cs, s_rs * s_sn, s_r * s_z};
      if (kind == 0) {
        absorbed = rabs(normal.x - rnd.x) < real(1e-8) && rabs(normal.y - rnd.y) < real(1e-8) &&
                   rabs(normal.z - rnd.z) < real(1e-8);
        rd = normal + rnd;
      } else {
        rd = dirbase + m_fuzz * rnd;
      }
      if (absorbed) {
        need_sample = true;
        --s_left;
        ++g.sample;
      } else {
#ifdef RTOW_FAST_MATH
        throughput = throughput * m_att;
#else
        P.stack[(size_t)nb * P.n_lanes + lane_g] = (uint32_t)mi;
#endif
        ++nb;
        --depth;
      }
    }
    stage_prio<kPrioStage>();
    const bool tracing = live && !need_sample;

    stamps.mark(RG_REGEN, __ballot(do_regen || do_scat));
    if constexpr (STAMPS) {
      stamps.trips += 1;
      if (t_empty != 0ull) trips_after_empty += 1;
      stamps.tail = t_empty != 0ull;
    }
    if constexpr (KERNEL != 3 && KERNEL != 4) {
      best.t = 0;
      best.prim = -1;
    }
    if constexpr (KERNEL == 4) {
      best = closest_hit_bvh4<LDS, STAMPS>(im4, sc, P, ro, rd, rtime, tracing, lane_g, nnode, nprim, stamps, best, w_cur, w_sa,
                                           P.walk_cap, P.walk_max_open);
    } else if constexpr (KERNEL == 3) {
      if constexpr (STAMPS) stamps.primary = __ballot(tracing && depth == P.max_child_rays);
      const RTOW_CONST TraceParams *kw = (const RTOW_CONST TraceParams *)__builtin_amdgcn_kernarg_segment_ptr();
      if constexpr ((SPEC & 3) != 0) asm volatile("" : "+s"(kw));
      best = closest_hit_grid<LDS, STAMPS, (SPEC & 3), (SPEC & (int)kSpecFlatY) != 0>(
          im, sc, ro, rd, rtime, tracing, nnode, nprim, stamps, best, t_resume, P.walk_cap, P.walk_max_open, P.leaf_votes,
          &kw->walk);
    } else if constexpr (KERNEL == 2) {
      best = closest_hit_bvh<LDS, STAMPS>(im, sc, ro, rd, rtime, tracing, nnode, nprim, stamps);
    } else if constexpr (KERNEL == 5) {
#ifndef RTOW_FAST_MATH
      if (tracing) best = closest_hit_reftree(sc, to_f64(ro), to_f64(rd), (double)rtime, nnode, nprim);
#endif
    } else {
      best = closest_hit_stream(sc, to_f64(ro), to_f64(rd), (double)rtime, tracing);
    }

    stamps.mark(RG_WALK, __ballot(tracing));
    bool arrived = tracing;
    if constexpr (KERNEL == 3) arrived = tracing && !(t_resume > 0.0f);
    if constexpr (KERNEL == 4) arrived = tracing && w_cur == 0x1fffffu;
    if (arrived) {
      ++nseg;
      if (best.prim >= 0) {
        if (depth <= 0)
          need_sample = true;
        else
          pending_hit = true;
      } else {
        const V3 unit = normalize(rd);
        const real t = real(0.5) * (unit.y + real(+1.0));
        V3 c = (real(1.0) - t) * V3{1, 1, 1} + t * V3{real(0.5), real(0.7), real(1.0)};
#ifdef RTOW_FAST_MATH
        c = throughput * c;
#else
        for (int q = nb - 1; q >= 0; --q) {
          const uint32_t smi = P.stack[(size_t)q * P.n_lanes + lane_g];
          if constexpr (KERNEL == 4) {
            const uint32_t mr = sc.b4_off_mats + 48u * smi;
            const vd2 a0 = im4.d2(mr), a1 = im4.d2(mr + 16u);
            c = V3{(real)a0.x, (real)a0.y, (real)a1.x} * c;
          } else if constexpr (KERNEL >= 2 && KERNEL <= 4) {
            const uint32_t mr = (KERNEL == 3 ? sc.g_off_mats : sc.off_mats) + 48u * smi;
            const double2 a0 = im.d2(mr), a1 = im.d2(mr + 16u);
            c = V3{(real)a0.x, (real)a0.y, (real)a1.x} * c;
          } else {
            const DevMaterial *m = sc.mats + smi;
            c = V3{(real)m->att[0], (real)m->att[1], (real)m->att[2]} * c;
          }
        }
#endif
        {
          V3d cd = to_f64(c);
          asm volatile("" : "+v"(cd.x), "+v"(cd.y), "+v"(cd.z));
          acc = acc + cd;
        }
        need_sample = true;
      }
      if (need_sample) {
        --s_left;
        ++g.sample;
      }
    }
    stamps.mark(RG_SHADE, __ballot(arrived));
  }
  if constexpr (STAMPS) {
    if (lane == 0)
    {
      const unsigned long long tend = __builtin_amdgcn_s_memrealtime();
      atomicAdd(&P.counters[4], tend - P.t_origin[0]);
      atomicMin(&P.counters[5], tend - P.t_origin[0]);
      atomicMax(&P.counters[6], tend - P.t_origin[0]);
      atomicAdd(&P.counters[7], t_empty - P.t_origin[0]);
      {
        const unsigned long long after = tend - t_empty;
        unsigned bin = (unsigned)(after / 20000ull);
        bin = bin > 5u ? 5u : bin;
        atomicAdd(&P.counters[17 + bin], 1ull);
        atomicMax(&P.counters[40], trips_after_empty);
        if (bin >= 2u) {
          atomicAdd(&P.counters[41], trips_after_empty);
          atomicAdd(&P.counters[42], after);
          atomicAdd(&P.counters[43], 1ull);
        }
      }
      for (int r = 0; r < RG_COUNT; ++r) atomicAdd(&P.counters[8 + r], stamps.t[r]);
      for (int r = 0; r < RG_COUNT; ++r) atomicAdd(&P.counters[29 + r], stamps.tt[r]);
      atomicAdd(&P.counters[37], trips_after_empty);
      atomicAdd(&P.counters[38], tend - t_empty);
      for (int r = 0; r < RG_COUNT; ++r) atomicAdd(&P.counters[23 + r], stamps.lt[r]);
      atomicAdd(&P.counters[34], stamps.step_lanes);
      atomicAdd(&P.counters[44], stamps.blocks);
      atomicAdd(&P.counters[36], stamps.block_lanes);
      atomicAdd(&P.counters[35], stamps.leaf_lanes);
      atomicAdd(&P.counters[45], stamps.iters_cam);
      atomicAdd(&P.counters[46], stamps.phases_cam);
      atomicAdd(&P.counters[13], stamps.iters);
      atomicAdd(&P.counters[14], stamps.trips);
      atomicAdd(&P.counters[15], stamps.phases);
    }
  }

#ifdef RTOW_TAILSTAT
  if (lane == 0 && P.spill != nullptr) {
    unsigned long long *ts = (unsigned long long *)P.spill + (size_t)((blockIdx.x * blockDim.x + threadIdx.x) >> 6) * 8;
    ts[0] = ts_start;
    ts[1] = ts_empty;
    ts[2] = __builtin_amdgcn_s_memrealtime();
    ts[3] = ts_trips;
    ts[4] = ts_trips_after;
    ts[5] = ts_live;
    ts[6] = ts_left;
    ts[7] = ts_pool;
  }
#endif
  unsigned long long t0 = nseg, t1 = nprim, t2 = nnode;
#pragma unroll
  for (int off = 32; off >= 1; off >>= 1) {
    t0 += __shfl_down(t0, off);
    t1 += __shfl_down(t1, off);
    t2 += __shfl_down(t2, off);
  }
  if (lane == 0) {
    atomicAdd(&P.counters[1], t0);
    if (KERNEL >= 2) {
      atomicAdd(&P.counters[2], t1);
      atomicAdd(&P.counters[3], t2);
    }
  }
}

#include "rtow_trace_sm4.h"

}

#include "rtow_kernel_launch.h"

template <int K, bool L, bool S, int SPEC = 0>
static KernelVariant<TraceParams> trace_kernel(unsigned lds_bytes) {
  return kernel_variant<RTOW_CAT(rtow_trace_, RTOW_SUFFIX)<K, L, S, SPEC>, TraceParams>(lds_bytes);
}
template <bool L, bool S>
static KernelVariant<TraceParams> trace4_kernel(unsigned lds_bytes) {
  return kernel_variant<RTOW_CAT(rtow_trace4_, RTOW_SUFFIX)<L, S>, TraceParams>(lds_bytes);
}

static KernelVariant<TraceParams> trace_variant(int kernel, unsigned lds_bytes, uint32_t spec, bool b4_full,
                                                bool b4_trips) {
  const bool lds = lds_bytes > 0;
  switch (kernel) {
    case 1: return trace_kernel<1, false, false>(lds_bytes);
    case 2: return lds ? trace_kernel<2, true, false>(lds_bytes) : trace_kernel<2, false, false>(0);
    case 3:
      if (lds && spec == kSpecStaticSpheres) return trace_kernel<3, true, false, 1>(lds_bytes);
      if (lds && spec == kSpecMovingSpheres) return trace_kernel<3, true, false, 2>(lds_bytes);
      if (lds && spec == (kSpecStaticSpheres | kSpecFlatY)) return trace_kernel<3, true, false, 1 | (int)kSpecFlatY>(lds_bytes);
      if (lds && spec == (kSpecMovingSpheres | kSpecFlatY)) return trace_kernel<3, true, false, 2 | (int)kSpecFlatY>(lds_bytes);
      return lds ? trace_kernel<3, true, false>(lds_bytes) : trace_kernel<3, false, false>(0);
    case 4:
      if (b4_trips) return b4_full ? trace_kernel<4, true, false>(lds_bytes) : trace_kernel<4, false, false>(lds_bytes);
      return b4_full ? trace4_kernel<true, false>(lds_bytes) : trace4_kernel<false, false>(lds_bytes);
    case 4 + 16:
      if (b4_trips) return b4_full ? trace_kernel<4, true, true>(lds_bytes) : trace_kernel<4, false, true>(lds_bytes);
      return b4_full ? trace4_kernel<true, true>(lds_bytes) : trace4_kernel<false, true>(lds_bytes);
#ifndef RTOW_FAST_MATH
    case 5: return trace_kernel<5, false, false>(0);
#endif
    case 2 + 16: return trace_kernel<2, true, true>(lds_bytes);
    case 3 + 16: return trace_kernel<3, true, true>(lds_bytes);
    default: return {};
  }
}

int RTOW_CAT(launch_trace_, RTOW_SUFFIX)(const TraceParams &p, int kernel, int grid, int block,
                                         unsigned lds_bytes, void *stream) {
  const KernelVariant<TraceParams> v = trace_variant(kernel, lds_bytes, p.spec, p.sc.b4_half == 0u, p.b4_trips != 0u);
  return v.fn ? v.launch(p, grid, block, v.lds_bytes, (hipStream_t)stream) : (int)hipErrorInvalidValue;
}

int RTOW_CAT(trace_occupancy_, RTOW_SUFFIX)(int kernel, int block, unsigned lds_bytes) {
  const KernelVariant<TraceParams> v = trace_variant(kernel, lds_bytes, kSpecGeneric, true, true);
  return resident_blocks(v.fn, block, v.lds_bytes, nullptr);
}

}
```

### raytracing-one-weekend_amd/csrc/rtow_trace_bvh.h

```cpp
#pragma once

template <bool LDS>
struct Image {
  const unsigned char *g;
  __device__ __forceinline__ float4 f4(uint32_t off) const {
    if constexpr (LDS)
      return *reinterpret_cast<const float4 *>(rtow_lds + off);
    else
      return *reinterpret_cast<const float4 *>(g + off);
  }
  __device__ __forceinline__ double2 d2(uint32_t off) const {
    if constexpr (LDS)
      return *reinterpret_cast<const double2 *>(rtow_lds + off);
    else
      return *reinterpret_cast<const double2 *>(g + off);
  }
  __device__ __forceinline__ uint32_t u32(uint32_t off) const {
    if constexpr (LDS)
      return *reinterpret_cast<const uint32_t *>(rtow_lds + off);
    else
      return *reinterpret_cast<const uint32_t *>(g + off);
  }
  __device__ __forceinline__ uint4 u4(uint32_t off) const {
    if constexpr (LDS)
// ... 2 lines not shown
      return *reinterpret_cast<const uint4 *>(g + off);
  }
  __device__ __forceinline__ double d1(uint32_t off) const {
    if constexpr (LDS)
      return *reinterpret_cast<const double *>(rtow_lds + off);
    else
      return *reinterpret_cast<const double *>(g + off);
  }
};

#if defined(RTOW_FAST_MATH) && !defined(RTOW_REAL_F32)
#define RTOW_UNIT_RAYS 1
#endif

__device__ __forceinline__ float round_up_f32(double t) { return (float)t * 1.00000048f; }
__device__ __forceinline__ float round_up_f32(float t) { return t; }

__device__ __forceinline__ float safe_inv(float d) {
  const float big = 1e30f;
  return __builtin_amdgcn_fmed3f(__builtin_amdgcn_rcpf(d), -big, big);
}

struct ImgOffsets {
  uint32_t ids, sph, mov, tri;
  uint32_t fat;
  uint32_t fat_stride;
  uint32_t sph32, mov32;
};

struct RayForms {
  V3 o, d;
  real a, inv_a, time;
  V3d o64, d64;
  double a64, inv_a64, time64;
  double tmin;
#ifdef RTOW_UNIT_RAYS
  bool unit;
  double od, oo;
  V3d o2;
#endif
};
__device__ __forceinline__ RayForms make_ray_forms(V3 o, V3 d, real time) {
  RayForms r;
  r.o = o;
  r.d = d;
  r.time = time;
  r.a = dot(d, d);
  r.inv_a = fast_rcp(r.a);
  r.o64 = to_f64(o);
  r.d64 = to_f64(d);
  r.time64 = (double)time;
#ifdef RTOW_REAL_F32
  r.a64 = dot(r.d64, r.d64);
  r.inv_a64 = fast_rcp(r.a64);
#else
  r.a64 = r.a;
  r.inv_a64 = r.inv_a;
#endif
  r.tmin = RTOW_TMIN;
#ifdef RTOW_UNIT_RAYS
  r.unit = false;
  r.od = r.oo = 0.0;
  r.o2 = V3d{0, 0, 0};
#endif
  return r;
}
#ifdef RTOW_UNIT_RAYS
__device__ __forceinline__ RayForms make_unit_ray_forms(V3d o, V3d du, double time, double len) {
  RayForms r;
  r.o = r.o64 = o;
  r.d = r.d64 = du;
  r.time = r.time64 = time;
  r.a = r.a64 = 1.0;
  r.inv_a = r.inv_a64 = 1.0;
  r.tmin = RTOW_TMIN * len;
  r.unit = true;
  r.od = dot(o, du);
  r.oo = dot(o, o);
  r.o2 = V3d{-2.0 * o.x, -2.0 * o.y, -2.0 * o.z};
  return r;
}
#endif

template <bool LDS, bool SMALL, int SPEC = 0, bool GRID = false>
__device__ __forceinline__ void leaf_test(const Image<LDS> &im, const DevScene &sc, ImgOffsets off,
                                          uint32_t first, uint32_t count, const RayForms &ray, Closest &best,
                                          uint32_t &nprim, int &last_id) {
#ifndef RTOW_REAL_F32
  if constexpr (SMALL) {
    if constexpr (SPEC == 1) __builtin_assume(off.fat != 0u && off.fat_stride == 48u);
    if constexpr (SPEC == 2) __builtin_assume(off.fat != 0u && off.fat_stride == 80u);
    if (off.fat != 0u) {
      if (off.fat_stride == 48u) {
#ifdef RTOW_UNIT_RAYS
        if (ray.unit) {
          for (uint32_t k = 0; k < count; ++k) {
            const uint32_t e = off.fat + 48u * (first + k);
            uint4 hd = im.u4(e);
            double2 p0 = im.d2(e + 16u);
            double cz = im.d1(e + 32u);
            asm volatile("" : "+v"(hd.x), "+v"(hd.z), "+v"(hd.w), "+v"(p0.x), "+v"(p0.y), "+v"(cz));
            const int id = (int)hd.x;
            if (id == last_id) continue;
            last_id = id;
            ++nprim;
            const double kk = __longlong_as_double((long long)(((unsigned long long)hd.w << 32) | hd.z));
            const double h = __builtin_fma(-p0.x, ray.d64.x, __builtin_fma(-p0.y, ray.d64.y, __builtin_fma(-cz, ray.d64.z, ray.od)));
            const double c = __builtin_fma(p0.x, ray.o2.x, __builtin_fma(p0.y, ray.o2.y, __builtin_fma(cz, ray.o2.z, ray.oo + kk)));
            const double disc = __builtin_fma(h, h, -c);
            if (disc >= 0.0) {
              const double sq = fast_sqrt_pos(disc);
              const double root1 = -h - sq, root2 = sq - h;
              const double root = root1 >= ray.tmin ? root1 : root2;
              if (root >= ray.tmin && root <= (double)best.t) {
                best.t = (real)root;
                best.prim = id;
              }
            }
          }
          return;
        }
#endif
        for (uint32_t k = 0; k < count; ++k) {
          const uint32_t e = off.fat + 48u * (first + k);
          const int id = (int)im.u32(e);
          double2 p0 = im.d2(e + 16u), p1 = im.d2(e + 32u);
          asm volatile("" : "+v"(p0.x), "+v"(p0.y), "+v"(p1.x), "+v"(p1.y));
          if (id == last_id) continue;
          last_id = id;
          ++nprim;
          sphere_test<double>(ray.o64, ray.d64, ray.a64, ray.inv_a64, p0.x, p0.y, p1.x, p1.y, id, ray.tmin, best);
        }
      } else {
        for (uint32_t k = 0; k < count; ++k) {
          const uint32_t e = off.fat + 80u * (first + k);
          const int id = (int)im.u32(e);
          double2 p0 = im.d2(e + 16u), p1 = im.d2(e + 32u), p2 = im.d2(e + 48u), p3 = im.d2(e + 64u);
          asm volatile("" : "+v"(p0.x), "+v"(p0.y), "+v"(p1.x), "+v"(p1.y), "+v"(p2.x), "+v"(p2.y), "+v"(p3.x));
          if (id == last_id) continue;
          last_id = id;
          ++nprim;
          const double cx = p0.x + ray.time64 * p1.y;
          const double cy = p0.y + ray.time64 * p2.x;
          const double cz = p1.x + ray.time64 * p2.y;
          sphere_test<double>(ray.o64, ray.d64, ray.a64, ray.inv_a64, cx, cy, cz, p3.x, id, ray.tmin, best);
        }
      }
      return;
    }
  }
#endif
  for (uint32_t k = 0; k < count; ++k) {
    const int id = (!SMALL && !GRID && sc.leaf_direct) ? (int)(first + k) : (int)im.u32(off.ids + 4u * (first + k));
    if constexpr (SPEC == 1) __builtin_assume(id < sc.n_sph);
    if constexpr (SPEC == 2) __builtin_assume(id < sc.n_sph + sc.n_mov);
    if (id == last_id) continue;
    last_id = id;
    ++nprim;
    if (id < sc.n_sph) {
#ifdef RTOW_REAL_F32
      if constexpr (SMALL) {
        const float4 p = im.f4(off.sph32 + 16u * (uint32_t)id);
        sphere_test<float>(ray.o, ray.d, ray.a, ray.inv_a, p.x, p.y, p.z, p.w, id, (float)ray.tmin, best);
        continue;
      }
#endif
      const uint32_t r = off.sph + 32u * (uint32_t)id;
      const double2 p0 = im.d2(r), p1 = im.d2(r + 16u);
      sphere_test<double>(ray.o64, ray.d64, ray.a64, ray.inv_a64, p0.x, p0.y, p1.x, p1.y, id, ray.tmin, best);
    } else if (id < sc.n_sph + sc.n_mov) {
#ifdef RTOW_REAL_F32
      if constexpr (SMALL) {
        const uint32_t r = off.mov32 + 32u * (uint32_t)(id - sc.n_sph);
        const float4 p0 = im.f4(r), p1 = im.f4(r + 16u);
        sphere_test<float>(ray.o, ray.d, ray.a, ray.inv_a, p0.x + ray.time * p0.w, p0.y + ray.time * p1.x,
                           p0.z + ray.time * p1.y, p1.z, id, (float)ray.tmin, best);
        continue;
      }
#endif
      const uint32_t r = off.mov + 64u * (uint32_t)(id - sc.n_sph);
      const double2 p0 = im.d2(r), p1 = im.d2(r + 16u), p2 = im.d2(r + 32u), p3 = im.d2(r + 48u);
      const double cx = p0.x + ray.time64 * p1.y;
      const double cy = p0.y + ray.time64 * p2.x;
      const double cz = p1.x + ray.time64 * p2.y;
      sphere_test<double>(ray.o64, ray.d64, ray.a64, ray.inv_a64, cx, cy, cz, p3.x, id, ray.tmin, best);
    } else {
#ifdef RTOW_REAL_F32
      const uint32_t r = off.tri + 48u * (uint32_t)(id - sc.n_sph - sc.n_mov);
      const float4 q0 = im.f4(r), q1 = im.f4(r + 16u), q2 = im.f4(r + 32u);
      triangle_test<float>(ray.o, ray.d, V3{q0.x, q0.y, q0.z}, V3{q0.w, q1.x, q1.y}, V3{q1.z, q1.w, q2.x},
                           V3{q2.y, q2.z, q2.w}, id, (float)ray.tmin, best);
#else
      const uint32_t r = off.tri + 96u * (uint32_t)(id - sc.n_sph - sc.n_mov);
      const double2 q0 = im.d2(r), q1 = im.d2(r + 16u), q2 = im.d2(r + 32u), q3 = im.d2(r + 48u),
                    q4 = im.d2(r + 64u), q5 = im.d2(r + 80u);
      triangle_test<double>(ray.o64, ray.d64, V3d{q0.x, q0.y, q1.x}, V3d{q1.y, q2.x, q2.y}, V3d{q3.x, q3.y, q4.x},
                            V3d{q4.y, q5.x, q5.y}, id, ray.tmin, best);
#endif
    }
  }
}

template <bool LDS, bool ST>
__device__ __forceinline__ Closest closest_hit_bvh(const Image<LDS> &im, const DevScene &sc, V3 o,
                                                   V3 d, real time, bool active, uint32_t &nnode,
                                                   uint32_t &nprim, Stamps<ST> &stamps) {
  Closest best;
  best.t = (real)__builtin_huge_val();
  best.prim = -1;
  const RayForms ray = make_ray_forms(o, d, time);
  const float ix = safe_inv((float)d.x), iy = safe_inv((float)d.y), iz = safe_inv((float)d.z);
  const float oix = (float)o.x * ix, oiy = (float)o.y * iy, oiz = (float)o.z * iz;
  const float tmin32 = 0.0009f;
  const float slack = 1.00002f;
  float tmax32 = __builtin_huge_valf();
  const uint32_t END = (uint32_t)sc.n_nodes;
  const ImgOffsets off = {sc.off_ids, sc.off_sph, sc.off_mov, sc.off_tri, 0u, 0u, sc.off_sph32, sc.off_mov32};
  int last_id = -1;
  uint32_t node = active ? 0u : END;
  uint32_t q0 = 0u, q1 = 0u, q2 = 0u, q3 = 0u;
  for (;;) {
    if constexpr (ST) stamps.iters += 1;
    if (node < END) {
      const float4 r0 = im.f4(node * 32u), r1 = im.f4(node * 32u + 16u);
      ++nnode;
      const float ax = fmaf(r0.x, ix, -oix), bx = fmaf(r0.w, ix, -oix);
      const float ay = fmaf(r0.y, iy, -oiy), by = fmaf(r1.x, iy, -oiy);
      const float az = fmaf(r0.z, iz, -oiz), bz = fmaf(r1.y, iz, -oiz);
      const float tnear = fmaxf(fmaxf(fminf(ax, bx), fminf(ay, by)), fmaxf(fminf(az, bz), tmin32));
      const float tfar = fminf(fminf(fmaxf(ax, bx), fmaxf(ay, by)), fminf(fmaxf(az, bz), tmax32));
      const bool hit = tnear <= tfar * slack;
      const uint32_t skip = __float_as_uint(r1.z), leaf = __float_as_uint(r1.w);
      if (hit && leaf != 0u) {
        if (q0 == 0u)
          q0 = leaf;
        else if (q1 == 0u)
          q1 = leaf;
        else if (q2 == 0u)
          q2 = leaf;
        else
          q3 = leaf;
      }
      node = (hit && leaf == 0u) ? node + 1u : skip;
    }
    const bool any_walking = __any(node < END);
    if (__any(q3 != 0u) || !any_walking) {
      stamps.mark(RG_WALK);
      if constexpr (ST) stamps.phases += 1;
      if (q0 != 0u) leaf_test<LDS, false>(im, sc, off, q0 >> 3, q0 & 7u, ray, best, nprim, last_id);
      q0 = q1;
      q1 = q2;
      q2 = q3;
      q3 = 0u;
      tmax32 = round_up_f32(best.t);
      stamps.mark(RG_LEAF);
      if (!any_walking && !__any(q0 != 0u)) break;
    }
  }
  return best;
}
```

### raytracing-one-weekend_amd/csrc/rtow_trace_bvh4.h

```cpp
#pragma once
constexpr uint32_t kRefNone = 0x1fffffu;
constexpr uint32_t kRefLeaf = 1u << 20;
constexpr uint32_t kRefPop = 0x1ffffeu;

template <bool FULL>
struct Bvh4Reader {
  const unsigned char *g;
  uint32_t lds_limit;
  uint32_t aux_src, aux_lds;
  template <class T>
  __device__ __forceinline__ T tri(uint32_t off) const {
    if constexpr (FULL)
      return lds_read<T>(off);
    else
      return glb_read<T>(g, off);
  }
  template <class T>
  __device__ __forceinline__ T rec(uint32_t off) const {
    if constexpr (FULL) {
      return lds_read<T>(off);
    } else {
      if (off >= aux_src) return lds_read<T>(aux_lds + (off - aux_src));
      return glb_read<T>(g, off);
    }
  }
  __device__ __forceinline__ vd2 t2(uint32_t off) const { return tri<vd2>(off); }
  __device__ __forceinline__ vd2 d2(uint32_t off) const { return rec<vd2>(off); }
  __device__ __forceinline__ uint32_t u32(uint32_t off) const { return rec<uint32_t>(off); }
};

struct Bvh4Ray {
  float ix, iy, iz, oix, oiy, oiz;
  float ixs, iys, izs, oixs, oiys, oizs;
  uint32_t nxo, nyo, nzo;
};
constexpr float kBvh4Slack = 1.00002f;
template <bool FULL>
__device__ __forceinline__ Bvh4Ray bvh4_ray(const DevScene &sc, V3 o, V3 d) {
  Bvh4Ray r;
  r.ix = safe_inv((float)d.x), r.iy = safe_inv((float)d.y), r.iz = safe_inv((float)d.z);
  if constexpr (!FULL) {
    r.oix = (float)(o.x - (real)sc.b4_c[0]) * r.ix, r.oiy = (float)(o.y - (real)sc.b4_c[1]) * r.iy,
    r.oiz = (float)(o.z - (real)sc.b4_c[2]) * r.iz;
    r.nxo = r.ix < 0.0f ? 8u : 0u, r.nyo = r.iy < 0.0f ? 24u : 16u, r.nzo = r.iz < 0.0f ? 40u : 32u;
    r.ix *= sc.b4_is[0], r.iy *= sc.b4_is[1], r.iz *= sc.b4_is[2];
  } else {
    r.oix = (float)o.x * r.ix, r.oiy = (float)o.y * r.iy, r.oiz = (float)o.z * r.iz;
    r.nxo = r.ix < 0.0f ? 16u : 0u, r.nyo = r.iy < 0.0f ? 48u : 32u, r.nzo = r.iz < 0.0f ? 80u : 64u;
  }
  r.ixs = r.ix * kBvh4Slack, r.iys = r.iy * kBvh4Slack, r.izs = r.iz * kBvh4Slack;
  r.oixs = r.oix * kBvh4Slack, r.oiys = r.oiy * kBvh4Slack, r.oizs = r.oiz * kBvh4Slack;
  return r;
}
constexpr uint32_t kBvh4StackStrideLog2 = 12u, kBvh4StackStride = 1u << kBvh4StackStrideLog2;
struct Bvh4Stack {
  uint32_t lds, end;
};
__device__ __forceinline__ Bvh4Stack bvh4_stack(const DevScene &sc) {
  Bvh4Stack st;
  st.lds = sc.b4_stack_base + 4u * threadIdx.x;
  st.end = st.lds + (sc.b4_stack_k << kBvh4StackStrideLog2);
  return st;
}

template <bool FULL, bool FOLD = true>
__device__ __forceinline__ void bvh4_step(const Bvh4Reader<FULL> &im, const TraceParams &P, const Bvh4Ray &r, float tmax32,
                                          Bvh4Stack st, uint32_t lane_g, uint32_t &cur, uint32_t &sa, uint32_t &q0,
                                          uint32_t &q1, uint32_t &nnode) {
  const float tmin32 = 0.0009f;
  const float tmaxs = FOLD ? tmax32 * kBvh4Slack : tmax32;
  const float fix = FOLD ? r.ixs : r.ix, fiy = FOLD ? r.iys : r.iy, fiz = FOLD ? r.izs : r.iz;
  const float foix = FOLD ? r.oixs : r.oix, foiy = FOLD ? r.oiys : r.oiy, foiz = FOLD ? r.oizs : r.oiz;
  if ((cur & kRefLeaf) != 0u && cur < kRefPop && q1 == kRefNone) {
    if (q0 == kRefNone)
      q0 = cur;
    else
      q1 = cur;
    cur = kRefPop;
  }
  if (cur == kRefPop) {
    if (sa == st.lds) {
      cur = kRefNone;
    } else {
      sa -= kBvh4StackStride;
      uint32_t e;
      if (sa < st.end)
        e = lds_read<uint32_t>(sa);
      else
        e = P.spill[(size_t)((sa - st.end) >> kBvh4StackStrideLog2) * P.n_lanes + lane_g];
      cur = (e >> 21) > (__float_as_uint(tmax32) >> 20) ? kRefPop : (e & 0x1fffffu);
    }
  }
  if (cur < kRefLeaf) {
    typedef typename std::conditional<FULL, vf4, vh4>::type planes_t;
    constexpr uint32_t kFar = FULL ? 16u : 8u, kChild = FULL ? 96u : 48u;
    const uint32_t nb = cur * (FULL ? 128u : 64u);
    planes_t nx, fx, ny, fy, nz, fz;
    vu4 cw;
    if (FULL || nb < im.lds_limit) {
      nx = lds_read<planes_t>(nb + r.nxo), fx = lds_read<planes_t>((nb + r.nxo) ^ kFar);
      ny = lds_read<planes_t>(nb + r.nyo), fy = lds_read<planes_t>((nb + r.nyo) ^ kFar);
      nz = lds_read<planes_t>(nb + r.nzo), fz = lds_read<planes_t>((nb + r.nzo) ^ kFar);
      cw = lds_read<vu4>(nb + kChild);
    } else if constexpr (!FULL) {
      const vu4 ax = glb_read<vu4>(im.g, nb), ay = glb_read<vu4>(im.g, nb + 16u), az = glb_read<vu4>(im.g, nb + 32u);
      cw = glb_read<vu4>(im.g, nb + kChild);
      const bool sx = (r.nxo & 8u) != 0u, sy = (r.nyo & 8u) != 0u, sz = (r.nzo & 8u) != 0u;
      typedef uint32_t vu2 __attribute__((ext_vector_type(2)));
      const vu2 nxu = {sx ? ax.z : ax.x, sx ? ax.w : ax.y}, fxu = {sx ? ax.x : ax.z, sx ? ax.y : ax.w};
      const vu2 nyu = {sy ? ay.z : ay.x, sy ? ay.w : ay.y}, fyu = {sy ? ay.x : ay.z, sy ? ay.y : ay.w};
      const vu2 nzu = {sz ? az.z : az.x, sz ? az.w : az.y}, fzu = {sz ? az.x : az.z, sz ? az.y : az.w};
      nx = __builtin_bit_cast(vh4, nxu), fx = __builtin_bit_cast(vh4, fxu);
      ny = __builtin_bit_cast(vh4, nyu), fy = __builtin_bit_cast(vh4, fyu);
      nz = __builtin_bit_cast(vh4, nzu), fz = __builtin_bit_cast(vh4, fzu);
    }
    ++nnode;
#define RTOW_SLAB(c, slot)                                                                                             \
  const float tn##slot = fmaxf(fmaxf(fmaf((float)nx.c, r.ix, -r.oix), fmaf((float)ny.c, r.iy, -r.oiy)),                \
                               fmaxf(fmaf((float)nz.c, r.iz, -r.oiz), tmin32));                                        \
  const float tf##slot = fminf(fminf(fmaf((float)fx.c, fix, -foix), fmaf((float)fy.c, fiy, -foiy)),                    \
                               fminf(fmaf((float)fz.c, fiz, -foiz), tmaxs));                                           \
  const bool h##slot = FOLD ? tn##slot <= tf##slot : tn##slot <= tf##slot * kBvh4Slack;                                \
  const uint32_t k##slot = h##slot ? ((__float_as_uint(tn##slot) & ~3u) | slot##u) : 0xffffffffu;
    RTOW_SLAB(x, 0)
    RTOW_SLAB(y, 1)
    RTOW_SLAB(z, 2)
    RTOW_SLAB(w, 3)
#undef RTOW_SLAB
    const uint32_t kmin = min(min(k0, k1), min(k2, k3));
    const uint32_t s = kmin & 3u;
    const uint32_t next = s == 0u ? cw.x : (s == 1u ? cw.y : (s == 2u ? cw.z : cw.w));
    cur = kmin == 0xffffffffu ? kRefPop : next;
#define RTOW_PUSH(slot, child)                                                                       \
  if (h##slot && s != slot##u) {                                                                     \
    const uint32_t e = ((__float_as_uint(tn##slot) >> 20) << 21) | child;                            \
    if (sa < st.end)                                                                                 \
      lds_write<uint32_t>(sa, e);                                                                    \
    else                                                                                             \
      P.spill[(size_t)((sa - st.end) >> kBvh4StackStrideLog2) * P.n_lanes + lane_g] = e;             \
    sa += kBvh4StackStride;                                                                          \
  }
    RTOW_PUSH(0, cw.x)
    RTOW_PUSH(1, cw.y)
    RTOW_PUSH(2, cw.z)
    RTOW_PUSH(3, cw.w)
#undef RTOW_PUSH
  }
}

template <bool FULL>
__device__ __forceinline__ void bvh4_leaf(const Bvh4Reader<FULL> &im, const DevScene &sc, uint32_t leaf, V3d o64, V3d d64,
                                          Closest &best, uint32_t &nprim) {
  const uint32_t first = (leaf & (kRefLeaf - 1u)) >> 2, count = (leaf & 3u) + 1u;
  for (uint32_t k = 0; k < count; ++k) {
    const uint32_t r = sc.b4_off_tri + 96u * (first + k);
    const vd2 t0 = im.t2(r), t1 = im.t2(r + 16u), t2 = im.t2(r + 32u), t3 = im.t2(r + 48u), t4 = im.t2(r + 64u),
              t5 = im.t2(r + 80u);
    ++nprim;
    triangle_test<double>(o64, d64, V3d{t0.x, t0.y, t1.x}, V3d{t1.y, t2.x, t2.y}, V3d{t3.x, t3.y, t4.x}, V3d{t4.y, t5.x, t5.y},
                          (int)(first + k), RTOW_TMIN, best);
  }
}
__device__ __forceinline__ bool bvh4_busy(uint32_t cur, uint32_t q1) {
  return cur != kRefNone && !((cur & kRefLeaf) != 0u && cur < kRefPop && q1 != kRefNone);
}

template <bool FULL, bool ST>
__device__ __forceinline__ Closest closest_hit_bvh4(const Bvh4Reader<FULL> &im, const DevScene &sc, const TraceParams &P,
                                                    V3 o, V3 d, real time, bool active, uint32_t lane_g, uint32_t &nnode,
                                                    uint32_t &nprim, Stamps<ST> &stamps, Closest best, uint32_t &w_cur,
                                                    uint32_t &w_sa, uint32_t cap, uint32_t max_open) {
  (void)time;
  const bool resumed = w_cur != kRefNone;
  if (!resumed) {
    best.t = (real)__builtin_huge_val();
    best.prim = -1;
  }
  const V3d o64 = to_f64(o), d64 = to_f64(d);
  const Bvh4Ray ray = bvh4_ray<FULL>(sc, o, d);
  const Bvh4Stack st = bvh4_stack(sc);
  float tmax32 = round_up_f32(best.t);
  uint32_t sa = resumed ? w_sa : st.lds;
  uint32_t cur = !active ? kRefNone : (resumed ? w_cur : 0u);
  uint32_t q0 = kRefNone, q1 = kRefNone;
  uint32_t trips = 0u;

  if constexpr (FULL) stage_prio<kPrioLeaf>();
  for (;;) {
    if constexpr (ST) {
      stamps.iters += 1;
      stamps.step_lanes += (unsigned long long)__popcll(__ballot(bvh4_busy(cur, q1)));
    }
    bvh4_step<FULL>(im, P, ray, tmax32, st, lane_g, cur, sa, q0, q1, nnode);
    const unsigned long long m_walking = __ballot(cur != kRefNone);
    const bool any_walking = m_walking != 0ull;
    ++trips;
    const bool suspend = any_walking && trips >= cap && (uint32_t)__popcll(m_walking) <= max_open;
    const unsigned long long m_pending = __ballot(q0 != kRefNone);
    if ((m_pending != 0ull && ((uint32_t)__popcll(m_pending) >= P.leaf_votes || __ballot(bvh4_busy(cur, q1)) == 0ull)) ||
        !any_walking || suspend) {
      stamps.mark(RG_WALK, __ballot(active));
      if constexpr (ST) {
        stamps.phases += 1;
        stamps.leaf_lanes += (unsigned long long)__popcll(m_pending);
      }
      if (q0 != kRefNone) bvh4_leaf<FULL>(im, sc, q0, o64, d64, best, nprim);
      q0 = q1;
      q1 = kRefNone;
      if (suspend && q0 != kRefNone) {
        bvh4_leaf<FULL>(im, sc, q0, o64, d64, best, nprim);
        q0 = kRefNone;
      }
      tmax32 = round_up_f32(best.t);
      stamps.mark(RG_LEAF, m_pending);
      if (suspend) {
        w_cur = cur;
        w_sa = sa;
        if constexpr (FULL) stage_prio<kPrioStage>();
        return best;
      }
      if (!any_walking && !__any(q0 != kRefNone)) break;
    }
  }
  w_cur = kRefNone;
  if constexpr (FULL) stage_prio<kPrioStage>();
  return best;
}
```

### raytracing-one-weekend_amd/csrc/rtow_trace_grid.h

```cpp
#pragma once
#include "rtow_dda_step.h"
template <bool LDS, bool ST, int SPEC = 0, bool FLAT = false>
__device__ __forceinline__ Closest closest_hit_grid(const Image<LDS> &im, const DevScene &sc, V3 o,
                                                    V3 d, real time, bool active, uint32_t &nnode,
                                                    uint32_t &nprim, Stamps<ST> &stamps, Closest best,
                                                    float &t_resume, uint32_t cap, uint32_t max_open,
                                                    uint32_t leaf_votes, const RTOW_CONST GridWalkConsts *wk = nullptr) {
  const bool resumed = t_resume > 0.0f;
  const float t_in = t_resume;
  if (!resumed) {
    best.t = (real)__builtin_huge_val();
    best.prim = -1;
  }
#ifdef RTOW_UNIT_RAYS
  const double a_ref = dot(d, d);
  const double inv_len = fast_rsqrt(a_ref), len = a_ref * inv_len;
  d = d * inv_len;
  const RayForms ray = make_unit_ray_forms(o, d, time, len);
  const float tmin32w = 0.0009f * (float)len;
#else
  const RayForms ray = make_ray_forms(o, d, time);
  const float tmin32w = 0.0009f;
#endif
  ImgOffsets off = {sc.g_off_ids, sc.g_off_sph, sc.g_off_mov, sc.g_off_tri, 0u, 0u, sc.g_off_sph32, sc.g_off_mov32};
  int last_id = -1;
  float gx, gy, gz, hx, hy, hz, cx, cy, cz, icx, icy, icz;
  int nx, ny, nxm1, nym1, nzm1, neg_nx, nxny, neg_nxny;
  [[maybe_unused]] int nz = 0;
  uint32_t n_large, lf, cells;
  if constexpr (SPEC != 0) {
    gx = wk->gx, gy = wk->gy, gz = wk->gz, hx = wk->hx, hy = wk->hy, hz = wk->hz;
    cx = wk->cx, cy = wk->cy, cz = wk->cz, icx = wk->icx, icy = wk->icy, icz = wk->icz;
    nx = wk->nx, ny = wk->ny, nxm1 = wk->nxm1, nym1 = wk->nym1, nzm1 = wk->nzm1;
    neg_nx = wk->neg_nx, nxny = wk->nxny, neg_nxny = wk->neg_nxny;
    n_large = wk->n_large, lf = wk->large_first, cells = wk->cells;
    off.fat = wk->fat;
    off.fat_stride = wk->fat_stride;
  } else {
    const RTOW_CONST float *hf = (const RTOW_CONST float *)sc.gblob;
    const RTOW_CONST int32_t *hi = (const RTOW_CONST int32_t *)sc.gblob;
    gx = hf[0], gy = hf[1], gz = hf[2];
    cx = hf[3], cy = hf[4], cz = hf[5];
    icx = hf[6], icy = hf[7], icz = hf[8];
    nx = hi[9], ny = hi[10], nz = hi[11];
    nxm1 = nx - 1, nym1 = ny - 1, nzm1 = nz - 1;
    neg_nx = -nx, nxny = nx * ny, neg_nxny = -(nx * ny);
    n_large = (uint32_t)hi[12];
    lf = ((uint32_t)hi[13] - off.ids) >> 2;
    cells = sc.g_off_cells;
    off.fat = (uint32_t)hi[14];
    off.fat_stride = (uint32_t)hi[15];
  }

  if (active && !resumed && n_large != 0u) {
    uint32_t k = 0;
    for (; k + 3 < n_large; k += 4) {
      int id[4];
#pragma unroll
      for (int j = 0; j < 4; ++j) id[j] = (int)im.u32(off.ids + 4u * (lf + k + j));
      if (SPEC == 1 || (id[0] < sc.n_sph && id[1] < sc.n_sph && id[2] < sc.n_sph && id[3] < sc.n_sph)) {
        double dd[4], hh[4];
#pragma unroll
        for (int j = 0; j < 4; ++j) {
          const uint32_t r = off.sph + 32u * (uint32_t)id[j];
          const double2 p0 = im.d2(r), p1 = im.d2(r + 16u);
          dd[j] = sphere_disc<double>(ray.o64, ray.d64, ray.a64, p0.x, p0.y, p1.x, p1.y, hh[j]);
        }
        nprim += 4u;
#pragma unroll
        for (int j = 0; j < 4; ++j) sphere_resolve<double>(dd[j], hh[j], ray.a64, ray.inv_a64, id[j], ray.tmin, best);
        last_id = id[3];
      } else {
        leaf_test<LDS, false, SPEC, true>(im, sc, off, lf + k, 4u, ray, best, nprim, last_id);
      }
    }
    for (; k + 1 < n_large; k += 2) {
      const int ia = (int)im.u32(off.ids + 4u * (lf + k)), ib = (int)im.u32(off.ids + 4u * (lf + k + 1));
      if (SPEC == 1 || (ia < sc.n_sph && ib < sc.n_sph)) {
        const uint32_t ra = off.sph + 32u * (uint32_t)ia, rb = off.sph + 32u * (uint32_t)ib;
        const double2 a0 = im.d2(ra), a1 = im.d2(ra + 16u), b0 = im.d2(rb), b1 = im.d2(rb + 16u);
        double ha, hb;
        const double da = sphere_disc<double>(ray.o64, ray.d64, ray.a64, a0.x, a0.y, a1.x, a1.y, ha);
        const double db = sphere_disc<double>(ray.o64, ray.d64, ray.a64, b0.x, b0.y, b1.x, b1.y, hb);
        nprim += 2u;
        sphere_resolve<double>(da, ha, ray.a64, ray.inv_a64, ia, ray.tmin, best);
        sphere_resolve<double>(db, hb, ray.a64, ray.inv_a64, ib, ray.tmin, best);
        last_id = ib;
      } else {
        leaf_test<LDS, false, SPEC, true>(im, sc, off, lf + k, 2u, ray, best, nprim, last_id);
      }
    }
    if (k < n_large) leaf_test<LDS, false, SPEC, true>(im, sc, off, lf + k, n_large - k, ray, best, nprim, last_id);
  }
  float tmax32 = round_up_f32(best.t);
  stage_prio<kPrioSetup>();

  const float dx = (float)d.x, dy = (float)d.y, dz = (float)d.z;
  const float ox = (float)o.x, oy = (float)o.y, oz = (float)o.z;
  const float ix = safe_inv(dx), iy = safe_inv(dy), iz = safe_inv(dz);
  const float oix = ox * ix, oiy = oy * iy, oiz = oz * iz;
  if constexpr (SPEC == 0) hx = fmaf((float)nx, cx, gx), hy = fmaf((float)ny, cy, gy), hz = fmaf((float)nz, cz, gz);
  const float ax = fmaf(gx, ix, -oix), bx = fmaf(hx, ix, -oix);
  const float ay = fmaf(gy, iy, -oiy), by = fmaf(hy, iy, -oiy);
  const float az = fmaf(gz, iz, -oiz), bz = fmaf(hz, iz, -oiz);
  const float t0 = fmaxf(fmaxf(fminf(ax, bx), fminf(ay, by)), fmaxf(fminf(az, bz), fmaxf(tmin32w, t_resume * 0.999999f)));
  const float t1 = fminf(fminf(fmaxf(ax, bx), fmaxf(ay, by)), fminf(fmaxf(az, bz), tmax32));
  bool walking = active && t0 <= t1 * 1.00002f;

  const bool fx = dx >= 0.0f, fy = dy >= 0.0f, fz = dz >= 0.0f;
  const float tdx = fabsf(cx * ix), tdz = fabsf(cz * iz);
  const float px = fmaf(t0, dx, ox), pz = fmaf(t0, dz, oz);
  int c0 = (int)floorf((px - gx) * icx), c2 = (int)floorf((pz - gz) * icz);
  c0 = min(max(c0, 0), nxm1);
  c2 = min(max(c2, 0), nzm1);
  typename DdaWalkOf<FLAT>::type w;
  w.tmx = fmaf(fmaf((float)(c0 + (fx ? 1 : 0)), cx, gx), ix, -oix);
  w.tmz = fmaf(fmaf((float)(c2 + (fz ? 1 : 0)), cz, gz), iz, -oiz);
  w.tdx = tdx, w.tdz = tdz;
  w.remx = fx ? nxm1 - c0 : c0, w.remz = fz ? nzm1 - c2 : c2;
  w.incx = fx ? 1 : -1;
  if constexpr (FLAT) {
    w.ty_exit = fy ? by : ay;
    w.incz = fz ? nx : neg_nx;
    w.idx = c2 * nx + c0;
  } else {
    const float py = fmaf(t0, dy, oy);
    int c1 = (int)floorf((py - gy) * icy);
    c1 = min(max(c1, 0), nym1);
    w.tmy = fmaf(fmaf((float)(c1 + (fy ? 1 : 0)), cy, gy), iy, -oiy);
    w.tdy = fabsf(cy * iy);
    w.remy = fy ? nym1 - c1 : c1;
    w.incy = fy ? nx : neg_nx, w.incz = fz ? nxny : neg_nxny;
    w.idx = (c2 * ny + c1) * nx + c0;
  }

  stage_prio<kPrioStage>();
  uint32_t q0 = 0u, q1 = 0u;
  float t_entry = t0;
// ... 62 lines not shown
```

### raytracing-one-weekend_amd/csrc/rtow_trace_hit.h

```cpp
#pragma once
struct Closest {
  real t;
  int prim;
};

__device__ __forceinline__ double rabs(double x) { return fabs(x); }
__device__ __forceinline__ float rabs(float x) { return fabsf(x); }

template <class T>
__device__ __forceinline__ T sphere_disc(Vec3<T> o, Vec3<T> d, T a, T cx, T cy, T cz, T r2, T &h) {
  Vec3<T> oc = {o.x - cx, o.y - cy, o.z - cz};
  h = dot(oc, d);
  T c = dot(oc, oc) - rabs(r2);
  return h * h - a * c;
}

template <class T>
__device__ __forceinline__ void sphere_resolve(T disc, T h, T a, T inv_a, int id, T tmin, Closest &best) {
  if (disc >= T(0.0)) {
#if defined(RTOW_FAST_MATH)
    const T sq = fast_sqrt_pos(disc);
    const T root1 = (-h - sq) * inv_a, root2 = (-h + sq) * inv_a;
    const T root = root1 >= tmin ? root1 : root2;
    if (root >= tmin && root <= (T)best.t) {
      best.t = (real)root;
      best.prim = id;
    }
#else
    (void)inv_a;
    const T sq = fast_sqrt(disc);
    T root = (-h - sq) / a;
    bool ok = true;
    if (root < tmin || root > (T)best.t) {
      root = (-h + sq) / a;
      if (root < tmin || root > (T)best.t) ok = false;
    }
    if (ok) {
      best.t = (real)root;
      best.prim = id;
    }
#endif
  }
}

template <class T>
__device__ __forceinline__ void sphere_test(Vec3<T> o, Vec3<T> d, T a, T inv_a, T cx, T cy, T cz, T r2, int id,
                                            T tmin, Closest &best) {
  T h;
  const T disc = sphere_disc(o, d, a, cx, cy, cz, r2, h);
  sphere_resolve(disc, h, a, inv_a, id, tmin, best);
}

template <class T>
__device__ __forceinline__ void triangle_test(Vec3<T> o, Vec3<T> d, Vec3<T> A, Vec3<T> e1, Vec3<T> e2, Vec3<T> n,
                                              int id, T tmin, Closest &best) {
  T det = -dot(d, n);
#if defined(RTOW_FAST_MATH) && !defined(RTOW_TRI_DIVIDE)
  {
    const Vec3<T> ao = o - A;
    const Vec3<T> dao = cross(ao, d);
    const T ud = dot(e2, dao), vd = -dot(e1, dao), td = dot(ao, n);
    if (det >= T(1e-6) && td >= tmin * det && td <= (T)best.t * det && ud >= T(0.0) && vd >= T(0.0) && (ud + vd) <= det) {
      best.t = (real)(td * fast_rcp(det));
      best.prim = id;
    }
    return;
  }
#endif
  T invdet = fast_rcp(det);
  Vec3<T> ao = o - A;
  Vec3<T> dao = cross(ao, d);
  T u = dot(e2, dao) * invdet;
  T v = -dot(e1, dao) * invdet;
  T t = dot(ao, n) * invdet;
  if (det >= T(1e-6) && t >= tmin && t <= (T)best.t && u >= T(0.0) && v >= T(0.0) && (u + v) <= T(1.0)) {
    best.t = (real)t;
    best.prim = id;
  }
}

#define RTOW_TMIN 0.001

constexpr uint32_t kStreamTile = 32u, kStreamTileBytes = kStreamTile * 96u;
__device__ __forceinline__ Closest closest_hit_stream(const DevScene &sc, V3d o, V3d d, double time, bool active) {
  Closest best;
  best.t = (real)__builtin_huge_val();
// ... 113 lines not shown
```

### raytracing-one-weekend_amd/csrc/rtow_walk_consts.h

```cpp
#pragma once

#if defined(__HIPCC__) || defined(__CUDACC__)
#define RTOW_WALK_FN __host__ __device__ inline
#else
#define RTOW_WALK_FN inline
#endif

struct alignas(64) GridWalkConsts {
  float gx, gy, gz;
  float hx, hy, hz;
  float cx, cz;
  float icx, icz;
  int nx, nxm1, nzm1;
  int neg_nx;
  unsigned cells;
  unsigned large_first;
  unsigned n_large;
  unsigned fat, fat_stride;
  int ny;
  float cy, icy;
  int nym1;
  int nxny, neg_nxny;
  int pad_[7];
};
static_assert(sizeof(GridWalkConsts) == 128, "two 64-byte lines");

RTOW_WALK_FN GridWalkConsts make_grid_walk_consts(const unsigned char *header, unsigned off_ids, unsigned off_cells) {
  float hf[9];
  int hi[3];
  unsigned hu[4];
  __builtin_memcpy(hf, header, 36);
  __builtin_memcpy(hi, header + 36, 12);
  __builtin_memcpy(hu, header + 48, 16);
  GridWalkConsts w{};
  w.gx = hf[0], w.gy = hf[1], w.gz = hf[2];
  w.hx = __builtin_fmaf((float)hi[0], hf[3], hf[0]);
  w.hy = __builtin_fmaf((float)hi[1], hf[4], hf[1]);
  w.hz = __builtin_fmaf((float)hi[2], hf[5], hf[2]);
  w.cx = hf[3], w.cy = hf[4], w.cz = hf[5];
  w.icx = hf[6], w.icy = hf[7], w.icz = hf[8];
  w.nx = hi[0], w.ny = hi[1];
  w.nxm1 = hi[0] - 1, w.nym1 = hi[1] - 1, w.nzm1 = hi[2] - 1;
  w.neg_nx = -hi[0];
  w.nxny = hi[0] * hi[1], w.neg_nxny = -(hi[0] * hi[1]);
  w.cells = off_cells;
  w.n_large = hu[0];
  w.large_first = (hu[1] - off_ids) >> 2;
  w.fat = hu[2], w.fat_stride = hu[3];
  return w;
}
```

### raytracing-one-weekend_amd/rtow.py

```python
from __future__ import annotations

import ctypes as C
import os
from pathlib import Path

import numpy as np

PKG_DIR = Path(__file__).resolve().parent
REPO_ROOT = PKG_DIR.parent
LIB_PATH = Path(os.environ.get("RTOW_LIB", PKG_DIR / "librtow.so"))

RTOW_ABI_VERSION = 9
RTOW_OK, RTOW_EINVAL, RTOW_ENODEV, RTOW_EHIP, RTOW_ENOSCENE, RTOW_EEMPTY, RTOW_ENOMEM = 0, -1, -2, -3, -4, -5, -6
MAT_LAMBERTIAN, MAT_METAL, MAT_DIELECTRIC = 0, 1, 2
PRIM_SPHERE, PRIM_MOVING_SPHERE, PRIM_TRIANGLE = 0, 1, 2
F64_STRICT, F64_FAST, F32 = 0, 1, 2
KERNEL_AUTO, KERNEL_BRUTE, KERNEL_BVH, KERNEL_GRID, KERNEL_BVH4, KERNEL_REFTREE = 0, 1, 2, 3, 4, 5
MAX_HITS = 8
MAX_NEAREST = 8
SPEC_GENERIC, SPEC_STATIC_SPHERES, SPEC_MOVING_SPHERES, SPEC_FLAT_Y = 0, 1, 2, 4
MODEL_OO, MODEL_VARIANT, MODEL_WORLD = 0, 1, 2
BUILDER_HOST_SAH, BUILDER_DEVICE_LBVH, BUILDER_AUTO = 0, 1, 2

d3 = C.c_double * 3
# ... 73 lines not shown
    ]


class Ray(C.Structure):
    _fields_ = [("origin", d3), ("time", C.c_double), ("direction", d3), ("tmax", C.c_double)]


class Hit(C.Structure):
    _fields_ = [
        ("t", C.c_double), ("point", d3), ("normal", d3),
        ("prim", C.c_int32), ("kind", C.c_int32), ("material", C.c_int32), ("front_face", C.c_int32),
    ]


class PointQuery(C.Structure):
    _fields_ = [("point", d3), ("time", C.c_double), ("max_dist", C.c_double), ("pad_", C.c_double)]


class PointHit(C.Structure):
    _fields_ = [
        ("dist", C.c_double), ("point", d3),
        ("prim", C.c_int32), ("kind", C.c_int32), ("material", C.c_int32), ("pad_", C.c_int32),
    ]


class Guide(C.Structure):
    _fields_ = [("albedo", d3), ("normal", d3), ("depth", C.c_double), ("hits", C.c_double)]


class RadianceParams(C.Structure):
    _fields_ = [("seed", C.c_uint64), ("samples_per_ray", C.c_int32), ("max_child_rays", C.c_int32),
                ("sample_first", C.c_uint32), ("pad_", C.c_int32)]


RAY_DTYPE = np.dtype([("origin", "<f8", (3,)), ("time", "<f8"), ("direction", "<f8", (3,)), ("tmax", "<f8")])
HIT_DTYPE = np.dtype([("t", "<f8"), ("point", "<f8", (3,)), ("normal", "<f8", (3,)), ("prim", "<i4"), ("kind", "<i4"),
                      ("material", "<i4"), ("front_face", "<i4")])

GUIDE_DTYPE = np.dtype([("albedo", "<f8", (3,)), ("normal", "<f8", (3,)), ("depth", "<f8"), ("hits", "<f8")])


POINT_QUERY_DTYPE = np.dtype([("point", "<f8", (3,)), ("time", "<f8"), ("max_dist", "<f8"), ("pad_", "<f8")])
POINT_HIT_DTYPE = np.dtype([("dist", "<f8"), ("point", "<f8", (3,)), ("prim", "<i4"), ("kind", "<i4"),
                            ("material", "<i4"), ("pad_", "<i4")])


def make_point_queries(points, time=0.0, max_dist=float("inf")):
    p = np.asarray(points, dtype=np.float64).reshape(-1, 3)
    q = np.empty(len(p), dtype=POINT_QUERY_DTYPE)
    q["point"] = p
    q["time"] = time
    q["max_dist"] = max_dist
    q["pad_"] = 0.0
    return q


def make_rays(origins, directions, time=0.0, tmax=float("inf")):
    o = np.asarray(origins, dtype=np.float64).reshape(-1, 3)
    d = np.asarray(directions, dtype=np.float64).reshape(-1, 3)
    r = np.empty(len(o), dtype=RAY_DTYPE)
    r["origin"] = o
    r["direction"] = d
    r["time"] = time
    r["tmax"] = tmax
    return r


EXPORTS = [
    "rtow_abi_version", "rtow_last_error", "rtow_ctx_create", "rtow_ctx_destroy",
    "rtow_scene_upload", "rtow_local_rows", "rtow_local_row_list", "rtow_render_device",
    "rtow_render", "rtow_host_scene_cover", "rtow_host_scene_obj", "rtow_host_scene_free",
    "rtow_host_rng_reset", "rtow_host_ppm", "rtow_host_free", "rtow_tonemap_device",
    "rtow_profile_collect", "rtow_debug_counters", "rtow_render_rgb8",
    "rtow_ctx_set_builder", "rtow_build_info", "rtow_debug_image", "rtow_render_multi",
    "rtow_debug_schedule", "rtow_host_scene_cover_model", "rtow_host_scene_obj_model",
    "rtow_multi_create", "rtow_multi_set_builder", "rtow_multi_upload", "rtow_multi_build_info",
    "rtow_multi_render", "rtow_multi_destroy", "rtow_host_reftree_info",
    "rtow_render_device_rgb8", "rtow_multi_render_rgb8", "rtow_multi_frame_breakdown",
    "rtow_intersect_device", "rtow_intersect", "rtow_occluded_device", "rtow_occluded",
    "rtow_scene_refit", "rtow_refit_info", "rtow_closest_point_device", "rtow_closest_point",
    "rtow_debug_tile_order", "rtow_radiance_device", "rtow_radiance",
    "rtow_camera_rays_device", "rtow_camera_rays", "rtow_camera_ray_count", "rtow_guides_device", "rtow_guides",
    "rtow_debug_last_spec", "rtow_first_hits_device", "rtow_first_hits", "rtow_nearest_device", "rtow_nearest",
]
MULTI_BREAKDOWN = ("total", "handoff_enqueue", "place_enqueue", "wait_and_copy", "wait_only", "dev_trace", "dev_gather",
                   "dev_place_copy")


class RtowError(RuntimeError):
    pass


_lib = None


def lib():
    global _lib
    if _lib is not None:
        return _lib
    try:
        import torch
    except ImportError:
        pass
    if not LIB_PATH.exists():
        raise RtowError(f"{LIB_PATH} is missing: run `python -c 'import __graft_entry__ as g; g.build()'`"
                        " (there is no CPU fallback)")
    L = C.CDLL(str(LIB_PATH))
    L.rtow_abi_version.restype = C.c_int
    L.rtow_last_error.restype = C.c_char_p
    L.rtow_ctx_create.argtypes = [C.c_int, C.POINTER(C.c_void_p)]
    L.rtow_ctx_destroy.argtypes = [C.c_void_p]
    L.rtow_ctx_destroy.restype = None
    L.rtow_scene_upload.argtypes = [C.c_void_p, C.POINTER(Scene)]
    L.rtow_local_rows.argtypes = [C.POINTER(Config)]
    L.rtow_local_row_list.argtypes = [C.POINTER(Config), _pi, C.c_int32]
    L.rtow_render_device.argtypes = [C.c_void_p, C.POINTER(Config), C.c_void_p, C.c_void_p,
                                     C.POINTER(Stats)]
    L.rtow_render.argtypes = [C.c_void_p, C.POINTER(Scene), C.POINTER(Config), _pd,
                              C.POINTER(Stats)]
    L.rtow_host_scene_cover.argtypes = [C.POINTER(HostConfig), C.POINTER(C.POINTER(Scene))]
    L.rtow_host_scene_obj.argtypes = [C.POINTER(HostConfig), C.c_char_p,
                                      C.POINTER(C.POINTER(Scene))]
    if hasattr(L, "rtow_host_scene_cover_model"):
        L.rtow_host_scene_cover_model.argtypes = [C.POINTER(HostConfig), C.c_int32, C.POINTER(C.POINTER(Scene))]
        L.rtow_host_scene_obj_model.argtypes = [C.POINTER(HostConfig), C.c_char_p, C.c_int32,
                                                C.POINTER(C.POINTER(Scene))]
    L.rtow_host_scene_free.argtypes = [C.POINTER(Scene)]
    L.rtow_host_scene_free.restype = None
    L.rtow_host_rng_reset.restype = None
    L.rtow_host_ppm.argtypes = [_pd, C.c_int32, C.c_int32, C.c_int32, C.POINTER(C.c_char_p),
                                C.POINTER(C.c_uint64)]
    L.rtow_host_free.argtypes = [C.c_void_p]
    L.rtow_host_free.restype = None
    L.rtow_tonemap_device.argtypes = [C.c_void_p, C.c_void_p, C.c_int64, C.c_int32, C.c_void_p, C.c_void_p]
    L.rtow_ctx_set_builder.argtypes = [C.c_void_p, C.c_int32]
    L.rtow_build_info.argtypes = [C.c_void_p, C.POINTER(BuildInfo)]
    L.rtow_render_multi.argtypes = [C.c_int32, _pi, C.POINTER(Scene), C.POINTER(Config), _pd, C.POINTER(Stats),
                                    C.c_int32]
    L.rtow_debug_image.argtypes = [C.c_void_p, C.c_int32, C.c_void_p, C.c_int64, C.POINTER(C.c_int64)]
    if hasattr(L, "rtow_host_reftree_info"):
        L.rtow_host_reftree_info.argtypes = [C.POINTER(Scene), C.POINTER(C.c_int32), C.POINTER(C.c_int32),
                                             C.POINTER(C.c_double)]
    if hasattr(L, "rtow_multi_create"):
        L.rtow_multi_create.argtypes = [C.c_int32, _pi, C.c_int32, C.POINTER(C.c_void_p)]
        L.rtow_multi_set_builder.argtypes = [C.c_void_p, C.c_int32]
        L.rtow_multi_upload.argtypes = [C.c_void_p, C.POINTER(Scene)]
        L.rtow_multi_build_info.argtypes = [C.c_void_p, C.POINTER(BuildInfo)]
        L.rtow_multi_render.argtypes = [C.c_void_p, C.POINTER(Config), _pd, C.POINTER(Stats)]
        L.rtow_multi_destroy.argtypes = [C.c_void_p]
        L.rtow_multi_destroy.restype = None
    if hasattr(L, "rtow_multi_render_rgb8"):
        L.rtow_multi_render_rgb8.argtypes = [C.c_void_p, C.POINTER(Config), C.c_void_p, C.POINTER(Stats)]
        L.rtow_render_device_rgb8.argtypes = [C.c_void_p, C.POINTER(Config), C.c_void_p, C.c_void_p, C.POINTER(Stats)]
    L.rtow_render_rgb8.argtypes = [C.c_void_p, C.POINTER(Scene), C.POINTER(Config), C.c_void_p, C.POINTER(Stats)]
    if hasattr(L, "rtow_intersect"):
        L.rtow_intersect_device.argtypes = [C.c_void_p, C.c_int32, C.c_int32, C.c_void_p, C.c_int64, C.c_void_p,
                                            C.c_void_p, C.POINTER(Stats)]
        L.rtow_intersect.argtypes = [C.c_void_p, C.c_int32, C.c_int32, C.c_void_p, C.c_int64, C.c_void_p,
                                     C.POINTER(Stats)]
    if hasattr(L, "rtow_occluded"):
        L.rtow_occluded_device.argtypes = [C.c_void_p, C.c_int32, C.c_int32, C.c_void_p, C.c_int64, C.c_void_p,
                                           C.c_void_p, C.POINTER(Stats)]
        L.rtow_occluded.argtypes = [C.c_void_p, C.c_int32, C.c_int32, C.c_void_p, C.c_int64, C.c_void_p,
                                    C.POINTER(Stats)]
    if hasattr(L, "rtow_first_hits"):
        L.rtow_first_hits_device.argtypes = [C.c_void_p, C.c_int32, C.c_int32, C.c_void_p, C.c_int64, C.c_int32, C.c_void_p,
                                             C.c_void_p, C.c_void_p, C.POINTER(Stats)]
        L.rtow_first_hits.argtypes = [C.c_void_p, C.c_int32, C.c_int32, C.c_void_p, C.c_int64, C.c_int32, C.c_void_p,
                                      C.c_void_p, C.POINTER(Stats)]
    if hasattr(L, "rtow_closest_point"):
        L.rtow_closest_point_device.argtypes = [C.c_void_p, C.c_int32, C.c_int32, C.c_void_p, C.c_int64, C.c_void_p,
                                                C.c_void_p, C.POINTER(Stats)]
        L.rtow_closest_point.argtypes = [C.c_void_p, C.c_int32, C.c_int32, C.c_void_p, C.c_int64, C.c_void_p,
                                         C.POINTER(Stats)]
    if hasattr(L, "rtow_nearest"):
        L.rtow_nearest_device.argtypes = [C.c_void_p, C.c_int32, C.c_int32, C.c_void_p, C.c_int64, C.c_int32, C.c_void_p,
                                          C.c_void_p, C.c_void_p, C.POINTER(Stats)]
        L.rtow_nearest.argtypes = [C.c_void_p, C.c_int32, C.c_int32, C.c_void_p, C.c_int64, C.c_int32, C.c_void_p,
                                   C.c_void_p, C.POINTER(Stats)]
    if hasattr(L, "rtow_radiance"):
        L.rtow_radiance_device.argtypes = [C.c_void_p, C.c_int32, C.c_int32, C.POINTER(RadianceParams), C.c_void_p, C.c_int64,
                                           C.c_void_p, C.c_void_p, C.c_void_p, C.POINTER(Stats)]
        L.rtow_radiance.argtypes = [C.c_void_p, C.c_int32, C.c_int32, C.POINTER(RadianceParams), C.c_void_p, C.c_int64,
                                    C.c_void_p, C.c_void_p, C.POINTER(Stats)]
    if hasattr(L, "rtow_guides"):
        L.rtow_camera_rays_device.argtypes = [C.c_void_p, C.POINTER(Config), C.c_void_p, C.c_void_p, C.c_void_p]
        L.rtow_camera_rays.argtypes = [C.c_void_p, C.POINTER(Config), C.c_void_p, C.c_void_p]
        L.rtow_camera_ray_count.argtypes = [C.POINTER(Config)]
        L.rtow_camera_ray_count.restype = C.c_int64
        L.rtow_guides_device.argtypes = [C.c_void_p, C.POINTER(Config), C.c_void_p, C.c_void_p, C.POINTER(Stats)]
        L.rtow_guides.argtypes = [C.c_void_p, C.POINTER(Config), C.c_void_p, C.POINTER(Stats)]
    if hasattr(L, "rtow_scene_refit"):
        L.rtow_scene_refit.argtypes = [C.c_void_p, C.POINTER(Scene)]
        L.rtow_refit_info.argtypes = [C.c_void_p, C.POINTER(RefitInfo)]
    L.rtow_profile_collect.argtypes = [C.c_void_p, C.POINTER(C.c_double), C.POINTER(C.c_int32)]
    if hasattr(L, "rtow_debug_schedule"):
        L.rtow_debug_schedule.argtypes = [C.c_void_p, C.POINTER(Config), C.POINTER(C.c_uint32), C.c_int32]
    if hasattr(L, "rtow_debug_tile_order"):
        L.rtow_debug_tile_order.argtypes = [C.POINTER(Scene), C.POINTER(Config), C.POINTER(C.c_uint32),
                                            C.POINTER(C.c_ubyte), C.c_int32, C.POINTER(C.c_int32),
                                            C.POINTER(C.c_int32), C.POINTER(C.c_int32)]
    if hasattr(L, "rtow_debug_last_spec"):
        L.rtow_debug_last_spec.argtypes = [C.c_void_p, C.POINTER(C.c_uint32)]
    ver = L.rtow_abi_version()
    if ver != RTOW_ABI_VERSION and not ("RTOW_LIB" in os.environ and ver >= 4):
        raise RtowError("librtow.so ABI version mismatch")
    _lib = L
    return L


def check(rc: int, what: str = "rtow"):
    if rc != 0:
        msg = lib().rtow_last_error()
        raise RtowError(f"{what} failed ({rc}): {msg.decode() if msg else ''}")


def image_height(width: int, aspect_ratio: float) -> int:
    return int(width / aspect_ratio)


def make_config(width, height, spp, nstreams=1, max_child_rays=50, seed=1, precision=F64_FAST,
                kernel=KERNEL_AUTO, rank=0, nranks=1, tile_rows=8, stream_first=0, stream_count=0,
                accumulate=0) -> Config:
    return Config(width, height, spp, nstreams, max_child_rays, precision, kernel, rank, nranks,
                  tile_rows, seed, stream_first, stream_count, accumulate, 0)


def spp_effective(cfg: Config) -> int:
    return cfg.samples_per_pixel // cfg.nstreams * cfg.nstreams


def local_rows(cfg: Config):
    L = lib()
    n = L.rtow_local_rows(C.byref(cfg))
    if n < 0:
        check(n, "rtow_local_rows")
    buf = (C.c_int32 * max(n, 1))()
    got = L.rtow_local_row_list(C.byref(cfg), buf, n)
    if got < 0:
        check(got, "rtow_local_row_list")
    return list(buf[:n])


class HostScene:

    def __init__(self, ptr):
        self.ptr = ptr

    @property
    def c(self) -> Scene:
        return self.ptr.contents

    @classmethod
    def cover(cls, nsqrt=11, aspect=1.5, moving=False, reset_rng=True, model=MODEL_OO):
        L = lib()
        if reset_rng:
            L.rtow_host_rng_reset()
        hc = HostConfig(nsqrt, aspect, int(moving))
        out = C.POINTER(Scene)()
        if model == MODEL_OO:
            check(L.rtow_host_scene_cover(C.byref(hc), C.byref(out)), "rtow_host_scene_cover")
        else:
            check(L.rtow_host_scene_cover_model(C.byref(hc), model, C.byref(out)), "rtow_host_scene_cover_model")
        return cls(out)

    @classmethod
    def obj(cls, path, aspect=16.0 / 9.0, reset_rng=True, model=MODEL_OO):
        L = lib()
        if reset_rng:
            L.rtow_host_rng_reset()
        hc = HostConfig(0, aspect, 0)
        out = C.POINTER(Scene)()
        if model == MODEL_OO:
            check(L.rtow_host_scene_obj(C.byref(hc), str(path).encode(), C.byref(out)), "rtow_host_scene_obj")
        else:
            check(L.rtow_host_scene_obj_model(C.byref(hc), str(path).encode(), model, C.byref(out)),
                  "rtow_host_scene_obj_model")
        return cls(out)

    def close(self):
        if self.ptr:
            lib().rtow_host_scene_free(self.ptr)
            self.ptr = None

    def __del__(self):
        try:
            self.close()
        except Exception:
            pass


def ppm_text(rgb_sums, width, height, spp_eff) -> bytes:
    import numpy as np

    a = np.ascontiguousarray(rgb_sums, dtype=np.float64)
    assert a.size == width * height * 3
    txt = C.c_char_p()
    n = C.c_uint64()
    L = lib()
    check(L.rtow_host_ppm(a.ctypes.data_as(_pd), width, height, spp_eff, C.byref(txt), C.byref(n)),
          "rtow_host_ppm")
    try:
        return C.string_at(txt, n.value)
    finally:
        L.rtow_host_free(txt)


class Context:

    def __init__(self, device_id: int = 0):
        self._h = C.c_void_p()
        check(lib().rtow_ctx_create(device_id, C.byref(self._h)), "rtow_ctx_create")
        self.device_id = device_id

    def upload(self, scene):
        s = scene.c if isinstance(scene, HostScene) else scene
        check(lib().rtow_scene_upload(self._h, C.byref(s)), "rtow_scene_upload")

    def refit(self, scene):
        s = scene.c if isinstance(scene, HostScene) else scene
        check(lib().rtow_scene_refit(self._h, C.byref(s)), "rtow_scene_refit")

    def refit_info(self) -> RefitInfo:
        ri = RefitInfo()
        check(lib().rtow_refit_info(self._h, C.byref(ri)), "rtow_refit_info")
        return ri

    def set_builder(self, builder: int):
        check(lib().rtow_ctx_set_builder(self._h, builder), "rtow_ctx_set_builder")

    def debug_image(self, which: int) -> bytes:
        n = C.c_int64()
        check(lib().rtow_debug_image(self._h, which, None, 0, C.byref(n)), "rtow_debug_image")
        buf = (C.c_ubyte * max(n.value, 1))()
        check(lib().rtow_debug_image(self._h, which, buf, n.value, C.byref(n)), "rtow_debug_image")
        return bytes(buf[:n.value])

    def last_spec(self) -> int:
        v = C.c_uint32()
        check(lib().rtow_debug_last_spec(self._h, C.byref(v)), "rtow_debug_last_spec")
        return int(v.value)

    def build_info(self) -> BuildInfo:
        bi = BuildInfo()
        check(lib().rtow_build_info(self._h, C.byref(bi)), "rtow_build_info")
        return bi

    def render_device(self, cfg: Config, d_ptr: int, stream: int = 0, want_stats=False):
        st = Stats() if want_stats else None
        check(lib().rtow_render_device(self._h, C.byref(cfg), C.c_void_p(d_ptr),
                                       C.c_void_p(stream), C.byref(st) if st is not None else None),
              "rtow_render_device")
        return st

    def tonemap_device(self, d_sums: int, n_values: int, spp_eff: int, d_rgb8: int, stream: int = 0):
        check(lib().rtow_tonemap_device(self._h, C.c_void_p(d_sums), n_values, spp_eff,
                                        C.c_void_p(d_rgb8), C.c_void_p(stream)), "rtow_tonemap_device")

    def render(self, scene, cfg: Config, into=None):
        import numpy as np

        s = scene.c if isinstance(scene, HostScene) else scene
        rows = lib().rtow_local_rows(C.byref(cfg))
        if rows < 0:
            check(rows, "rtow_local_rows")
        out = np.zeros((rows, cfg.image_width, 3), dtype=np.float64) if into is None else into
        st = Stats()
        check(lib().rtow_render(self._h, C.byref(s), C.byref(cfg), out.ctypes.data_as(_pd),
                                C.byref(st)), "rtow_render")
        return out, st

    def render_rgb8(self, scene, cfg: Config, want_stats=True):
        import numpy as np

        s = scene.c if isinstance(scene, HostScene) else scene
        rows = lib().rtow_local_rows(C.byref(cfg))
        if rows < 0:
            check(rows, "rtow_local_rows")
        out = np.zeros((rows, cfg.image_width, 3), dtype=np.uint8)
        st = Stats() if want_stats else None
        check(lib().rtow_render_rgb8(self._h, C.byref(s), C.byref(cfg), out.ctypes.data_as(C.c_void_p),
                                     C.byref(st) if st is not None else None), "rtow_render_rgb8")
        return out, st

    def render_device_rgb8(self, cfg: Config, d_ptr: int, stream: int = 0, want_stats=False):
        st = Stats() if want_stats else None
        check(lib().rtow_render_device_rgb8(self._h, C.byref(cfg), C.c_void_p(d_ptr), C.c_void_p(stream),
                                            C.byref(st) if st is not None else None), "rtow_render_device_rgb8")
        return st

    def intersect(self, rays, precision=F64_FAST, kernel=KERNEL_AUTO, want_stats=False):
        r = np.ascontiguousarray(rays, dtype=RAY_DTYPE).reshape(-1)
        hits = np.empty(len(r), dtype=HIT_DTYPE)
        st = Stats() if want_stats else None
        check(lib().rtow_intersect(self._h, precision, kernel, r.ctypes.data_as(C.c_void_p), len(r),
                                   hits.ctypes.data_as(C.c_void_p), C.byref(st) if st is not None else None),
              "rtow_intersect")
        return (hits, st) if want_stats else hits

    def intersect_device(self, d_rays: int, n: int, d_hits: int, precision=F64_FAST, kernel=KERNEL_AUTO,
                         stream: int = 0, want_stats=False):
        st = Stats() if want_stats else None
        check(lib().rtow_intersect_device(self._h, precision, kernel, C.c_void_p(d_rays), n, C.c_void_p(d_hits),
                                          C.c_void_p(stream), C.byref(st) if st is not None else None),
              "rtow_intersect_device")
        return st

    def occluded(self, rays, precision=F64_FAST, kernel=KERNEL_AUTO, want_stats=False):
        r = np.ascontiguousarray(rays, dtype=RAY_DTYPE).reshape(-1)
        out = np.empty(len(r), dtype=np.uint8)
        st = Stats() if want_stats else None
        check(lib().rtow_occluded(self._h, precision, kernel, r.ctypes.data_as(C.c_void_p), len(r),
                                  out.ctypes.data_as(C.c_void_p), C.byref(st) if st is not None else None),
              "rtow_occluded")
        occ = out.view(np.bool_)
        return (occ, st) if want_stats else occ

    def occluded_device(self, d_rays: int, n: int, d_occluded: int, precision=F64_FAST, kernel=KERNEL_AUTO,
                        stream: int = 0, want_stats=False):
        st = Stats() if want_stats else None
        check(lib().rtow_occluded_device(self._h, precision, kernel, C.c_void_p(d_rays), n, C.c_void_p(d_occluded),
                                         C.c_void_p(stream), C.byref(st) if st is not None else None),
              "rtow_occluded_device")
        return st

# ... 204 lines not shown
```

Before: 16950.

## Skip walk counters when stats are off and preload large-sphere head into scalar regs

```diff
diff --git a/include/rtow.h b/include/rtow.h
--- a/include/rtow.h
+++ b/include/rtow.h
@@ -157,6 +157,10 @@
 int rtow_debug_schedule(rtow_ctx *ctx, const rtow_config_t *cfg, uint32_t *out_pairs, int32_t capacity_pairs);
 
 int rtow_debug_last_spec(rtow_ctx *ctx, uint32_t *out_spec);
+
+int rtow_debug_last_counted(rtow_ctx *ctx, uint32_t *out_counted);
+
+int rtow_debug_walk_consts(rtow_ctx *ctx, void *out, int32_t capacity_bytes, int32_t *out_bytes);
 
 int rtow_debug_tile_order(const rtow_scene_t *scene, const rtow_config_t *cfg, uint32_t *table_out, unsigned char *empty_out,
                           int32_t capacity, int32_t *n_empty, int32_t *tile_w_log2, int32_t *tile_h_log2);
diff --git a/raytracing-one-weekend_amd/csrc/rtow_capi.cpp b/raytracing-one-weekend_amd/csrc/rtow_capi.cpp
--- a/raytracing-one-weekend_amd/csrc/rtow_capi.cpp
+++ b/raytracing-one-weekend_amd/csrc/rtow_capi.cpp
@@ -809,9 +809,11 @@
   if (slot >= 0) HIPCHK(hipEventRecord(c->ev[slot][0], st));
   int launch_kernel = kernel;
   if (image_kernel && lds_bytes > 0 && c->knobs.stamps) launch_kernel = kernel + 16;
-  int lrc = strict ? rtow::launch_trace_strict(P, launch_kernel, (int)grid, block, lds_bytes, st)
-            : f32  ? rtow::launch_trace_f32(P, launch_kernel, (int)grid, block, lds_bytes, st)
-                   : rtow::launch_trace_fast(P, launch_kernel, (int)grid, block, lds_bytes, st);
+  const bool want_count = stats != nullptr || c->knobs.count_always;
+  bool counted = true;
+  int lrc = strict ? rtow::launch_trace_strict(P, launch_kernel, (int)grid, block, lds_bytes, st, want_count, &counted)
+            : f32  ? rtow::launch_trace_f32(P, launch_kernel, (int)grid, block, lds_bytes, st, want_count, &counted)
+                   : rtow::launch_trace_fast(P, launch_kernel, (int)grid, block, lds_bytes, st, want_count, &counted);
 #ifdef RTOW_TAILSTAT
   if (const char *path = std::getenv("RTOW_TAILSTAT_OUT")) {
     HIPCHK(hipStreamSynchronize(st));
@@ -825,6 +827,7 @@
 #endif
   if (lrc != 0) return fail(RTOW_EHIP, "trace kernel launch failed: %s", hipGetErrorString((hipError_t)lrc));
   c->last_spec = (int64_t)P.spec;
+  c->last_counted = counted ? 1 : 0;
   if (slot >= 0) {
     HIPCHK(hipEventRecord(c->ev[slot][1], st));
     c->ev_count++;
@@ -1413,6 +1416,21 @@
   if (!c || !out_spec) return fail(RTOW_EINVAL, "NULL argument");
   if (c->last_spec < 0) return fail(RTOW_ENOSCENE, "no launch yet");
   *out_spec = (uint32_t)c->last_spec;
+  return RTOW_OK;
+}
+
+int rtow_debug_last_counted(rtow_ctx *c, uint32_t *out_counted) {
+  if (!c || !out_counted) return fail(RTOW_EINVAL, "NULL argument");
+  if (c->last_counted < 0) return fail(RTOW_ENOSCENE, "no launch yet");
+  *out_counted = (uint32_t)c->last_counted;
+  return RTOW_OK;
+}
+
+int rtow_debug_walk_consts(rtow_ctx *c, void *out, int32_t capacity_bytes, int32_t *out_bytes) {
+  if (!c || !out_bytes || capacity_bytes < 0 || (!out && capacity_bytes > 0)) return fail(RTOW_EINVAL, "NULL argument");
+  if (!c->have_scene) return fail(RTOW_ENOSCENE, "no scene uploaded");
+  *out_bytes = (int32_t)sizeof c->grid_walk;
+  if (capacity_bytes > 0) std::memcpy(out, &c->grid_walk, std::min<size_t>((size_t)capacity_bytes, sizeof c->grid_walk));
   return RTOW_OK;
 }
 
diff --git a/raytracing-one-weekend_amd/csrc/rtow_ctx.h b/raytracing-one-weekend_amd/csrc/rtow_ctx.h
--- a/raytracing-one-weekend_amd/csrc/rtow_ctx.h
+++ b/raytracing-one-weekend_amd/csrc/rtow_ctx.h
@@ -114,6 +114,7 @@
   bool stream_scalar = false;
   bool no_spec = false;
   bool no_flat = false;
+  bool count_always = false;
   bool tile_order = true;
   int empty_levels = 3;
   int tail_bound = 0;
@@ -168,6 +169,7 @@
     empty_levels = std::min(std::max(geti("RTOW_EMPTY_LEVELS", 3), 1), 16);
     no_spec = std::getenv("RTOW_NO_SPEC") != nullptr;
     no_flat = std::getenv("RTOW_NO_FLAT") != nullptr;
+    count_always = geti("RTOW_COUNT_ALWAYS", 0) != 0;
     stream_scalar = std::getenv("RTOW_STREAM_SCALAR") != nullptr;
     if (const char *e = std::getenv("RTOW_PLOC_RADIUS")) ploc_radius = std::min(std::max(std::atoi(e), 0), 64);
     if (const char *e = std::getenv("RTOW_DEVICE_TREE"))
@@ -198,6 +200,7 @@
   int32_t grid_ny = 0;
   GridWalkConsts grid_walk{};
   int64_t last_spec = -1;
+  int last_counted = -1;
   bool have_grid = false;
   uint32_t blob_bytes = 0;
   long long bvh_nodes = 0;
diff --git a/raytracing-one-weekend_amd/csrc/rtow_device.h b/raytracing-one-weekend_amd/csrc/rtow_device.h
--- a/raytracing-one-weekend_amd/csrc/rtow_device.h
+++ b/raytracing-one-weekend_amd/csrc/rtow_device.h
@@ -127,11 +127,11 @@
 };
 
 int launch_trace_strict(const TraceParams &p, int kernel, int grid, int block, unsigned lds_bytes,
-                        void *stream);
+                        void *stream, bool count = true, bool *counted = nullptr);
 int launch_trace_fast(const TraceParams &p, int kernel, int grid, int block, unsigned lds_bytes,
-                      void *stream);
+                      void *stream, bool count = true, bool *counted = nullptr);
 int launch_trace_f32(const TraceParams &p, int kernel, int grid, int block, unsigned lds_bytes,
-                     void *stream);
+                     void *stream, bool count = true, bool *counted = nullptr);
 int trace_occupancy_strict(int kernel, int block, unsigned lds_bytes);
 int trace_occupancy_fast(int kernel, int block, unsigned lds_bytes);
 int trace_occupancy_f32(int kernel, int block, unsigned lds_bytes);
diff --git a/raytracing-one-weekend_amd/csrc/rtow_scene.cpp b/raytracing-one-weekend_amd/csrc/rtow_scene.cpp
--- a/raytracing-one-weekend_amd/csrc/rtow_scene.cpp
+++ b/raytracing-one-weekend_amd/csrc/rtow_scene.cpp
@@ -197,11 +197,21 @@
   bvh4_set_frame(c, img4.map_c, img4.map_s);
 }
 
-static void grid_resident(rtow_ctx *c, const rtow::GridImage &gimg) {
+static int grid_resident(rtow_ctx *c, const rtow::GridImage &gimg, int n_sph) {
   c->have_grid = gimg.ok;
   c->grid_fat_stride = (gimg.ok && gimg.off_fat) ? gimg.fat_stride : 0u;
   c->grid_ny = gimg.ok ? gimg.n[1] : 0;
   c->grid_walk = gimg.ok ? make_grid_walk_consts(gimg.header, gimg.off_ids, gimg.off_cells) : GridWalkConsts{};
+  if (gimg.ok && c->grid_walk.n_large != 0u && gimg.off_fat != 0u) {
+    uint32_t head[kWalkLargeFast] = {};
+    const size_t n = std::min<size_t>(c->grid_walk.n_large, kWalkLargeFast) * sizeof(uint32_t);
+    const size_t off_large = (size_t)gimg.off_ids + 4u * (size_t)c->grid_walk.large_first;
+    if (gimg.blob.size() >= off_large + n)
+      std::memcpy(head, gimg.blob.data() + off_large, n);
+    else
+      HIPCHK(hipMemcpy(head, (const unsigned char *)c->gblob.p + off_large, n, hipMemcpyDeviceToHost));
+    fill_large_head(c->grid_walk, head, n_sph, gimg.off_sph);
+  }
   c->gblob_bytes = gimg.ok ? (uint32_t)gimg.total_bytes : 0u;
   rtow::DevScene &ds = c->ds;
   ds.gblob = (const unsigned char *)c->gblob.p;
@@ -215,6 +225,7 @@
     d->g_off_cells = gimg.off_cells;
     d->g_off_ids = gimg.off_ids;
   }
+  return RTOW_OK;
 }
 
 static void image32_resident(rtow::DevScene &d32, bool grid, const Image32 *im, const void *dev, size_t bytes) {
@@ -569,7 +580,7 @@
   if ((rc = build_grid(c, s->camera, rec, need, gimg, grid_on_device))) return rc;
   const double t_grid1 = now_ms();
   if (gimg.ok && !grid_on_device && (rc = upload(c->gblob, gimg.blob))) return rc;
-  grid_resident(c, gimg);
+  if ((rc = grid_resident(c, gimg, s->n_spheres))) return rc;
   publish_dev_scene(c, s, trees);
   c->ds32 = c->ds;
   if ((need & kNeedF32) && (rc = build_f32_images(c, rec, trees, gimg, grid_on_device))) return rc;
@@ -894,7 +905,7 @@
     rec.tri.resize((size_t)nt * 12);
     if ((rc = grid_device_build(c, s->camera, rec, gimg))) return rc;
   }
-  grid_resident(c, gimg);
+  if ((rc = grid_resident(c, gimg, ns))) return rc;
   if (!(c->built & kNeedF32)) return RTOW_OK;
   if (!gimg.ok) {
     image32_resident(c->ds32, true, nullptr, nullptr, 0);
diff --git a/raytracing-one-weekend_amd/csrc/rtow_trace_body.h b/raytracing-one-weekend_amd/csrc/rtow_trace_body.h
--- a/raytracing-one-weekend_amd/csrc/rtow_trace_body.h
+++ b/raytracing-one-weekend_amd/csrc/rtow_trace_body.h
@@ -220,7 +220,7 @@
   return !absorbed;
 }
 
-template <int KERNEL, bool LDS, bool STAMPS = false, int SPEC = 0>
+template <int KERNEL, bool LDS, bool STAMPS = false, int SPEC = 0, bool COUNT = true>
 __global__ void __launch_bounds__(KERNEL >= 2 && KERNEL <= 4 ? 1024 : 256)
     RTOW_CAT(rtow_trace_, RTOW_SUFFIX)(const TraceParams P) {
   const DevScene &sc = P.sc;
@@ -248,7 +248,12 @@
   V3 throughput = {1, 1, 1};
 #endif
   Rng g = {0, 0, 0};
-  uint32_t nseg = 0, nnode = 0, nprim = 0;
+#ifdef RTOW_TAILSTAT
+  constexpr bool kCount = true;
+#else
+  constexpr bool kCount = COUNT || STAMPS;
+#endif
+  WalkCount<kCount> nseg, nnode, nprim;
   [[maybe_unused]] float t_resume = 0.0f;
   [[maybe_unused]] uint32_t w_cur = 0x1fffffu, w_sa = 0u;
   Closest best;
@@ -697,7 +702,7 @@
       best = closest_hit_bvh<LDS, STAMPS>(im, sc, ro, rd, rtime, tracing, nnode, nprim, stamps);
     } else if constexpr (KERNEL == 5) {
 #ifndef RTOW_FAST_MATH
-      if (tracing) best = closest_hit_reftree(sc, to_f64(ro), to_f64(rd), (double)rtime, nnode, nprim);
+      if (tracing) best = closest_hit_reftree(sc, to_f64(ro), to_f64(rd), (double)rtime, nnode.n, nprim.n);
 #endif
     } else {
       best = closest_hit_stream(sc, to_f64(ro), to_f64(rd), (double)rtime, tracing);
@@ -801,18 +806,20 @@
     ts[7] = ts_pool;
   }
 #endif
-  unsigned long long t0 = nseg, t1 = nprim, t2 = nnode;
+  if constexpr (kCount) {
+    unsigned long long t0 = nseg.value(), t1 = nprim.value(), t2 = nnode.value();
 #pragma unroll
-  for (int off = 32; off >= 1; off >>= 1) {
-    t0 += __shfl_down(t0, off);
-    t1 += __shfl_down(t1, off);
-    t2 += __shfl_down(t2, off);
-  }
-  if (lane == 0) {
-    atomicAdd(&P.counters[1], t0);
-    if (KERNEL >= 2) {
-      atomicAdd(&P.counters[2], t1);
-      atomicAdd(&P.counters[3], t2);
+    for (int off = 32; off >= 1; off >>= 1) {
+      t0 += __shfl_down(t0, off);
+      t1 += __shfl_down(t1, off);
+      t2 += __shfl_down(t2, off);
+    }
+    if (lane == 0) {
+      atomicAdd(&P.counters[1], t0);
+      if (KERNEL >= 2) {
+        atomicAdd(&P.counters[2], t1);
+        atomicAdd(&P.counters[3], t2);
+      }
     }
   }
 }
@@ -823,9 +830,16 @@
 
 #include "rtow_kernel_launch.h"
 
-template <int K, bool L, bool S, int SPEC = 0>
+template <int K, bool L, bool S, int SPEC = 0, bool COUNT = true>
 static KernelVariant<TraceParams> trace_kernel(unsigned lds_bytes) {
-  return kernel_variant<RTOW_CAT(rtow_trace_, RTOW_SUFFIX)<K, L, S, SPEC>, TraceParams>(lds_bytes);
+  return kernel_variant<RTOW_CAT(rtow_trace_, RTOW_SUFFIX)<K, L, S, SPEC, COUNT>, TraceParams>(lds_bytes);
+}
+template <int K, bool L, int SPEC = 0>
+static KernelVariant<TraceParams> trace_kernel_by_count(unsigned lds_bytes, bool count) {
+#ifndef RTOW_REAL_F32
+  if (!count) return trace_kernel<K, L, false, SPEC, false>(lds_bytes);
+#endif
+  return trace_kernel<K, L, false, SPEC, true>(lds_bytes);
 }
 template <bool L, bool S>
 static KernelVariant<TraceParams> trace4_kernel(unsigned lds_bytes) {
@@ -833,19 +847,27 @@
 }
 
 static KernelVariant<TraceParams> trace_variant(int kernel, unsigned lds_bytes, uint32_t spec, bool b4_full,
-                                                bool b4_trips) {
+                                                bool b4_trips, bool count = true, bool *counted = nullptr) {
   const bool lds = lds_bytes > 0;
+  bool dummy;
+  bool &cnt = counted ? *counted : dummy;
+  cnt = true;
+#ifndef RTOW_REAL_F32
+  const bool has_nocount = (kernel == 3 && lds && (spec & 3u) != 0u) || (kernel == 4 && b4_trips);
+  if (has_nocount) cnt = count;
+#endif
   switch (kernel) {
     case 1: return trace_kernel<1, false, false>(lds_bytes);
     case 2: return lds ? trace_kernel<2, true, false>(lds_bytes) : trace_kernel<2, false, false>(0);
     case 3:
-      if (lds && spec == kSpecStaticSpheres) return trace_kernel<3, true, false, 1>(lds_bytes);
-      if (lds && spec == kSpecMovingSpheres) return trace_kernel<3, true, false, 2>(lds_bytes);
-      if (lds && spec == (kSpecStaticSpheres | kSpecFlatY)) return trace_kernel<3, true, false, 1 | (int)kSpecFlatY>(lds_bytes);
-      if (lds && spec == (kSpecMovingSpheres | kSpecFlatY)) return trace_kernel<3, true, false, 2 | (int)kSpecFlatY>(lds_bytes);
+      if (lds && spec == kSpecStaticSpheres) return trace_kernel_by_count<3, true, 1>(lds_bytes, cnt);
+      if (lds && spec == kSpecMovingSpheres) return trace_kernel_by_count<3, true, 2>(lds_bytes, cnt);
+      if (lds && spec == (kSpecStaticSpheres | kSpecFlatY)) return trace_kernel_by_count<3, true, 1 | (int)kSpecFlatY>(lds_bytes, cnt);
+      if (lds && spec == (kSpecMovingSpheres | kSpecFlatY)) return trace_kernel_by_count<3, true, 2 | (int)kSpecFlatY>(lds_bytes, cnt);
+      cnt = true;
       return lds ? trace_kernel<3, true, false>(lds_bytes) : trace_kernel<3, false, false>(0);
     case 4:
-      if (b4_trips) return b4_full ? trace_kernel<4, true, false>(lds_bytes) : trace_kernel<4, false, false>(lds_bytes);
+      if (b4_trips) return b4_full ? trace_kernel_by_count<4, true>(lds_bytes, cnt) : trace_kernel_by_count<4, false>(lds_bytes, cnt);
       return b4_full ? trace4_kernel<true, false>(lds_bytes) : trace4_kernel<false, false>(lds_bytes);
     case 4 + 16:
       if (b4_trips) return b4_full ? trace_kernel<4, true, true>(lds_bytes) : trace_kernel<4, false, true>(lds_bytes);
@@ -860,8 +882,9 @@
 }
 
 int RTOW_CAT(launch_trace_, RTOW_SUFFIX)(const TraceParams &p, int kernel, int grid, int block,
-                                         unsigned lds_bytes, void *stream) {
-  const KernelVariant<TraceParams> v = trace_variant(kernel, lds_bytes, p.spec, p.sc.b4_half == 0u, p.b4_trips != 0u);
+                                         unsigned lds_bytes, void *stream, bool count, bool *counted) {
+  const KernelVariant<TraceParams> v =
+      trace_variant(kernel, lds_bytes, p.spec, p.sc.b4_half == 0u, p.b4_trips != 0u, count, counted);
   return v.fn ? v.launch(p, grid, block, v.lds_bytes, (hipStream_t)stream) : (int)hipErrorInvalidValue;
 }
 
diff --git a/raytracing-one-weekend_amd/csrc/rtow_trace_bvh.h b/raytracing-one-weekend_amd/csrc/rtow_trace_bvh.h
--- a/raytracing-one-weekend_amd/csrc/rtow_trace_bvh.h
+++ b/raytracing-one-weekend_amd/csrc/rtow_trace_bvh.h
@@ -108,10 +108,10 @@
 }
 #endif
 
-template <bool LDS, bool SMALL, int SPEC = 0, bool GRID = false>
+template <bool LDS, bool SMALL, int SPEC = 0, bool GRID = false, class CN = uint32_t>
 __device__ __forceinline__ void leaf_test(const Image<LDS> &im, const DevScene &sc, ImgOffsets off,
                                           uint32_t first, uint32_t count, const RayForms &ray, Closest &best,
-                                          uint32_t &nprim, int &last_id) {
+                                          CN &nprim, int &last_id) {
 #ifndef RTOW_REAL_F32
   if constexpr (SMALL) {
     if constexpr (SPEC == 1) __builtin_assume(off.fat != 0u && off.fat_stride == 48u);
@@ -227,10 +227,10 @@
   }
 }
 
-template <bool LDS, bool ST>
+template <bool LDS, bool ST, class CN = uint32_t>
 __device__ __forceinline__ Closest closest_hit_bvh(const Image<LDS> &im, const DevScene &sc, V3 o,
-                                                   V3 d, real time, bool active, uint32_t &nnode,
-                                                   uint32_t &nprim, Stamps<ST> &stamps) {
+                                                   V3 d, real time, bool active, CN &nnode,
+                                                   CN &nprim, Stamps<ST> &stamps) {
   Closest best;
   best.t = (real)__builtin_huge_val();
   best.prim = -1;
diff --git a/raytracing-one-weekend_amd/csrc/rtow_trace_bvh4.h b/raytracing-one-weekend_amd/csrc/rtow_trace_bvh4.h
--- a/raytracing-one-weekend_amd/csrc/rtow_trace_bvh4.h
+++ b/raytracing-one-weekend_amd/csrc/rtow_trace_bvh4.h
@@ -63,10 +63,10 @@
   return st;
 }
 
-template <bool FULL, bool FOLD = true>
+template <bool FULL, bool FOLD = true, class CN = uint32_t>
 __device__ __forceinline__ void bvh4_step(const Bvh4Reader<FULL> &im, const TraceParams &P, const Bvh4Ray &r, float tmax32,
                                           Bvh4Stack st, uint32_t lane_g, uint32_t &cur, uint32_t &sa, uint32_t &q0,
-                                          uint32_t &q1, uint32_t &nnode) {
+                                          uint32_t &q1, CN &nnode) {
   const float tmin32 = 0.0009f;
   const float tmaxs = FOLD ? tmax32 * kBvh4Slack : tmax32;
   const float fix = FOLD ? r.ixs : r.ix, fiy = FOLD ? r.iys : r.iy, fiz = FOLD ? r.izs : r.iz;
@@ -148,9 +148,9 @@
   }
 }
 
-template <bool FULL>
+template <bool FULL, class CN = uint32_t>
 __device__ __forceinline__ void bvh4_leaf(const Bvh4Reader<FULL> &im, const DevScene &sc, uint32_t leaf, V3d o64, V3d d64,
-                                          Closest &best, uint32_t &nprim) {
+                                          Closest &best, CN &nprim) {
   const uint32_t first = (leaf & (kRefLeaf - 1u)) >> 2, count = (leaf & 3u) + 1u;
   for (uint32_t k = 0; k < count; ++k) {
     const uint32_t r = sc.b4_off_tri + 96u * (first + k);
@@ -165,10 +165,10 @@
   return cur != kRefNone && !((cur & kRefLeaf) != 0u && cur < kRefPop && q1 != kRefNone);
 }
 
-template <bool FULL, bool ST>
+template <bool FULL, bool ST, class CN = uint32_t>
 __device__ __forceinline__ Closest closest_hit_bvh4(const Bvh4Reader<FULL> &im, const DevScene &sc, const TraceParams &P,
-                                                    V3 o, V3 d, real time, bool active, uint32_t lane_g, uint32_t &nnode,
-                                                    uint32_t &nprim, Stamps<ST> &stamps, Closest best, uint32_t &w_cur,
+                                                    V3 o, V3 d, real time, bool active, uint32_t lane_g, CN &nnode,
+                                                    CN &nprim, Stamps<ST> &stamps, Closest best, uint32_t &w_cur,
                                                     uint32_t &w_sa, uint32_t cap, uint32_t max_open) {
   (void)time;
   const bool resumed = w_cur != kRefNone;
diff --git a/raytracing-one-weekend_amd/csrc/rtow_trace_grid.h b/raytracing-one-weekend_amd/csrc/rtow_trace_grid.h
--- a/raytracing-one-weekend_amd/csrc/rtow_trace_grid.h
+++ b/raytracing-one-weekend_amd/csrc/rtow_trace_grid.h
@@ -1,9 +1,9 @@
 #pragma once
 #include "rtow_dda_step.h"
-template <bool LDS, bool ST, int SPEC = 0, bool FLAT = false>
+template <bool LDS, bool ST, int SPEC = 0, bool FLAT = false, class CN = uint32_t>
 __device__ __forceinline__ Closest closest_hit_grid(const Image<LDS> &im, const DevScene &sc, V3 o,
-                                                    V3 d, real time, bool active, uint32_t &nnode,
-                                                    uint32_t &nprim, Stamps<ST> &stamps, Closest best,
+                                                    V3 d, real time, bool active, CN &nnode,
+                                                    CN &nprim, Stamps<ST> &stamps, Closest best,
                                                     float &t_resume, uint32_t cap, uint32_t max_open,
                                                     uint32_t leaf_votes, const RTOW_CONST GridWalkConsts *wk = nullptr) {
   const bool resumed = t_resume > 0.0f;
@@ -28,6 +28,9 @@
   int nx, ny, nxm1, nym1, nzm1, neg_nx, nxny, neg_nxny;
   [[maybe_unused]] int nz = 0;
   uint32_t n_large, lf, cells;
+  constexpr bool kLargeHead = SPEC == 2;
+  [[maybe_unused]] uint32_t nf = 0u, lrec[4] = {0u, 0u, 0u, 0u};
+  [[maybe_unused]] int lid[4] = {-1, -1, -1, -1};
   if constexpr (SPEC != 0) {
     gx = wk->gx, gy = wk->gy, gz = wk->gz, hx = wk->hx, hy = wk->hy, hz = wk->hz;
     cx = wk->cx, cy = wk->cy, cz = wk->cz, icx = wk->icx, icy = wk->icy, icz = wk->icz;
@@ -36,6 +39,13 @@
     n_large = wk->n_large, lf = wk->large_first, cells = wk->cells;
     off.fat = wk->fat;
     off.fat_stride = wk->fat_stride;
+    if constexpr (kLargeHead) {
+      nf = wk->n_large_fast;
+#pragma unroll
+      for (int j = 0; j < 4; ++j) lrec[j] = wk->large_rec[j], lid[j] = (int)wk->large_id[j];
+      asm volatile("" : "+s"(nf), "+s"(lrec[0]), "+s"(lrec[1]), "+s"(lrec[2]), "+s"(lrec[3]), "+s"(lid[0]), "+s"(lid[1]),
+                   "+s"(lid[2]), "+s"(lid[3]));
+    }
   } else {
     const RTOW_CONST float *hf = (const RTOW_CONST float *)sc.gblob;
     const RTOW_CONST int32_t *hi = (const RTOW_CONST int32_t *)sc.gblob;
@@ -54,6 +64,35 @@
 
   if (active && !resumed && n_large != 0u) {
     uint32_t k = 0;
+    if constexpr (kLargeHead) {
+      double dd[4], hh[4];
+      if (nf == 4u) {
+#pragma unroll
+        for (int j = 0; j < 4; ++j) {
+          const double2 p0 = im.d2(lrec[j]), p1 = im.d2(lrec[j] + 16u);
+          dd[j] = sphere_disc<double>(ray.o64, ray.d64, ray.a64, p0.x, p0.y, p1.x, p1.y, hh[j]);
+        }
+        nprim += 4u;
+#pragma unroll
+        for (int j = 0; j < 4; ++j) sphere_resolve<double>(dd[j], hh[j], ray.a64, ray.inv_a64, lid[j], ray.tmin, best);
+        last_id = lid[3];
+      } else if (nf != 0u) {
+#pragma unroll
+        for (int j = 0; j < 3; ++j)
+          if ((uint32_t)j < nf) {
+            const double2 p0 = im.d2(lrec[j]), p1 = im.d2(lrec[j] + 16u);
+            dd[j] = sphere_disc<double>(ray.o64, ray.d64, ray.a64, p0.x, p0.y, p1.x, p1.y, hh[j]);
+          }
+        nprim += nf;
+#pragma unroll
+        for (int j = 0; j < 3; ++j)
+          if ((uint32_t)j < nf) {
+            sphere_resolve<double>(dd[j], hh[j], ray.a64, ray.inv_a64, lid[j], ray.tmin, best);
+            last_id = lid[j];
+          }
+      }
+      k = nf;
+    }
     for (; k + 3 < n_large; k += 4) {
       int id[4];
 #pragma unroll
diff --git a/raytracing-one-weekend_amd/csrc/rtow_trace_hit.h b/raytracing-one-weekend_amd/csrc/rtow_trace_hit.h
--- a/raytracing-one-weekend_amd/csrc/rtow_trace_hit.h
+++ b/raytracing-one-weekend_amd/csrc/rtow_trace_hit.h
@@ -2,6 +2,20 @@
 struct Closest {
   real t;
   int prim;
+};
+
+template <bool COUNT>
+struct WalkCount {
+  uint32_t n = 0;
+  __device__ __forceinline__ WalkCount &operator++() { return ++n, *this; }
+  __device__ __forceinline__ WalkCount &operator+=(uint32_t k) { return n += k, *this; }
+  __device__ __forceinline__ uint32_t value() const { return n; }
+};
+template <>
+struct WalkCount<false> {
+  __device__ __forceinline__ WalkCount &operator++() { return *this; }
+  __device__ __forceinline__ WalkCount &operator+=(uint32_t) { return *this; }
+  __device__ __forceinline__ uint32_t value() const { return 0u; }
 };
 
 __device__ __forceinline__ double rabs(double x) { return fabs(x); }
diff --git a/raytracing-one-weekend_amd/csrc/rtow_walk_consts.h b/raytracing-one-weekend_amd/csrc/rtow_walk_consts.h
--- a/raytracing-one-weekend_amd/csrc/rtow_walk_consts.h
+++ b/raytracing-one-weekend_amd/csrc/rtow_walk_consts.h
@@ -22,8 +22,16 @@
   int nym1;
   int nxny, neg_nxny;
   int pad_[7];
+  unsigned large_rec[4];
+  unsigned large_id[4];
+  unsigned n_large_fast;
+  int pad2_[7];
 };
-static_assert(sizeof(GridWalkConsts) == 128, "two 64-byte lines");
+static_assert(sizeof(GridWalkConsts) == 192, "three 64-byte lines");
+static_assert(__builtin_offsetof(GridWalkConsts, large_rec) == 128 && __builtin_offsetof(GridWalkConsts, large_id) == 144 &&
+                  __builtin_offsetof(GridWalkConsts, n_large_fast) == 160,
+              "GridWalkConsts: the large list's head");
+constexpr unsigned kWalkLargeFast = 4;
 
 RTOW_WALK_FN GridWalkConsts make_grid_walk_consts(const unsigned char *header, unsigned off_ids, unsigned off_cells) {
   float hf[9];
@@ -49,3 +57,13 @@
   w.fat = hu[2], w.fat_stride = hu[3];
   return w;
 }
+
+RTOW_WALK_FN void fill_large_head(GridWalkConsts &w, const unsigned *large_ids, int n_sph, unsigned off_sph) {
+  const unsigned n = w.n_large < kWalkLargeFast ? w.n_large : kWalkLargeFast;
+  unsigned k = 0;
+  for (; k < n && large_ids[k] < (unsigned)n_sph; ++k) {
+    w.large_id[k] = large_ids[k];
+    w.large_rec[k] = off_sph + 32u * large_ids[k];
+  }
+  w.n_large_fast = k;
+}
diff --git a/raytracing-one-weekend_amd/rtow.py b/raytracing-one-weekend_amd/rtow.py
--- a/raytracing-one-weekend_amd/rtow.py
+++ b/raytracing-one-weekend_amd/rtow.py
@@ -179,6 +179,7 @@
     "rtow_debug_tile_order", "rtow_radiance_device", "rtow_radiance",
     "rtow_camera_rays_device", "rtow_camera_rays", "rtow_camera_ray_count", "rtow_guides_device", "rtow_guides",
     "rtow_debug_last_spec", "rtow_first_hits_device", "rtow_first_hits", "rtow_nearest_device", "rtow_nearest",
+    "rtow_debug_last_counted", "rtow_debug_walk_consts",
 ]
 MULTI_BREAKDOWN = ("total", "handoff_enqueue", "place_enqueue", "wait_and_copy", "wait_only", "dev_trace", "dev_gather",
                    "dev_place_copy")
@@ -299,6 +300,10 @@
                                             C.POINTER(C.c_int32), C.POINTER(C.c_int32)]
     if hasattr(L, "rtow_debug_last_spec"):
         L.rtow_debug_last_spec.argtypes = [C.c_void_p, C.POINTER(C.c_uint32)]
+    if hasattr(L, "rtow_debug_last_counted"):
+        L.rtow_debug_last_counted.argtypes = [C.c_void_p, C.POINTER(C.c_uint32)]
+    if hasattr(L, "rtow_debug_walk_consts"):
+        L.rtow_debug_walk_consts.argtypes = [C.c_void_p, C.c_void_p, C.c_int32, C.POINTER(C.c_int32)]
     ver = L.rtow_abi_version()
     if ver != RTOW_ABI_VERSION and not ("RTOW_LIB" in os.environ and ver >= 4):
         raise RtowError("librtow.so ABI version mismatch")
@@ -438,6 +443,18 @@
         check(lib().rtow_debug_last_spec(self._h, C.byref(v)), "rtow_debug_last_spec")
         return int(v.value)
 
+    def last_counted(self) -> bool:
+        v = C.c_uint32()
+        check(lib().rtow_debug_last_counted(self._h, C.byref(v)), "rtow_debug_last_counted")
+        return bool(v.value)
+
+    def walk_consts(self):
+        n = C.c_int32()
+        check(lib().rtow_debug_walk_consts(self._h, None, 0, C.byref(n)), "rtow_debug_walk_consts")
+        buf = (C.c_uint32 * (n.value // 4))()
+        check(lib().rtow_debug_walk_consts(self._h, buf, n.value, C.byref(n)), "rtow_debug_walk_consts")
+        return np.frombuffer(bytes(buf), dtype=np.uint32)
+
     def build_info(self) -> BuildInfo:
         bi = BuildInfo()
         check(lib().rtow_build_info(self._h, C.byref(bi)), "rtow_build_info")
```

New measurement: 17350, median of 6. +2.4%, better.
